# BUBLET/uav-airvision

Hardware: AMD Instinct MI355X
Metric: stereo frames/sec (LK+stereo+MSCKF-update) at 752x480 (higher is better)
Workload: dtype u8/int32 windows, f32 normal equations

## Files before the change

### include/airvision.h

```cpp
#ifndef AIRVISION_H
#define AIRVISION_H

#include <stddef.h>
#include <stdint.h>

#ifdef __cplusplus
extern "C" {
#endif

#define AV_OK            0
#define AV_E_INVALID    -1
#define AV_E_HIP        -2
#define AV_E_CAPACITY   -3
#define AV_E_NODEVICE   -4
#define AV_E_NUMERIC    -5

#define AV_MAX_LEVELS    5
#define AV_PYR_BORDER   16
#define AV_MAX_IMAGE_PIXELS (1 << 24)

const char* av_last_error(void);
const char* av_version(void);
int av_device_count(void);

typedef struct av_pyr_layout {
    int32_t levels;
    int32_t w[AV_MAX_LEVELS], h[AV_MAX_LEVELS];
    int32_t pitch[AV_MAX_LEVELS];
    int64_t offset[AV_MAX_LEVELS];
    int64_t bytes;
} av_pyr_layout;

int av_pyramid_layout(int w, int h, int levels, av_pyr_layout* out);

int av_pyramid_build(const uint8_t* img_dev, int64_t img_stride, int n_img, int w, int h, int levels,
                     uint8_t* pyr_dev, int64_t pyr_stride, void* stream);

int av_lk_track(const uint8_t* pyrI_dev, const uint8_t* pyrJ_dev, int64_t pyr_stride, int n_set,
                int w, int h, int levels,
                const float* prev_dev, float* next_dev, uint8_t* status_dev, const int32_t* count_dev, int cap,
                int win, int max_iter, double eps, double min_eig_threshold, void* stream);

int av_fast_detect(const uint8_t* img_dev, int64_t img_stride, const uint8_t* mask_dev, int64_t mask_stride,
                   int n_img, int w, int h, int threshold, uint32_t* kp_dev, int32_t* count_dev, int cap,
                   void* stream);
int av_fast_detect_wide(const uint8_t* img_dev, int64_t img_stride, const uint8_t* mask_dev, int64_t mask_stride,
                        int n_img, int w, int h, int threshold, uint32_t* kp_dev, int32_t* count_dev, int cap,
                        void* stream);

int av_undistort_points(const double* pts_dev, int n, const double* intr, const double* dist, const double* R,
                        double* out_dev, void* stream);
int av_distort_points(const double* pts_dev, int n, const double* intr, const double* dist,
                      double* out_dev, void* stream);

#define AV_DISTORTION_RADTAN 0
#define AV_DISTORTION_EQUIDISTANT 1
int av_undistort_points_model(const double* pts_dev, int n, const double* intr, const double* dist, const double* R, int model,
                              double* out_dev, void* stream);
int av_distort_points_model(const double* pts_dev, int n, const double* intr, const double* dist, int model,
                            double* out_dev, void* stream);

typedef struct av_frontend_config {
    int32_t width, height;
    int32_t grid_row, grid_col;
    int32_t grid_min_feature_num;
    int32_t grid_max_feature_num;
    int32_t fast_threshold;
    int32_t lk_win;
    int32_t lk_levels;
    int32_t lk_max_iter;
    int32_t max_corners;
    int32_t flags;
    double  lk_eps;
    double  lk_min_eig;
    double  stereo_threshold;
    double  cam0_intrinsics[4], cam0_distortion[4];
    double  cam1_intrinsics[4], cam1_distortion[4];
    double  R_cam0_imu[9], R_cam1_imu[9];
    double  R0to1[9];
    double  E[9];
    double  norm_unit;
    int32_t cam0_distortion_model;
    int32_t cam1_distortion_model;
    double  ransac_threshold;
    double  ransac_success_probability;
    uint32_t ransac_seed;
    int32_t reserved0;
    double  clahe_clip_limit;
    int32_t clahe_tiles_x, clahe_tiles_y;
    int32_t pixel_format;
    int32_t gray16_shift;
    int32_t image_downscale;
    int32_t reserved1;
} av_frontend_config;

typedef struct av_frontend av_frontend;

int  av_frontend_create(const av_frontend_config* cfg, int n_streams, int device, av_frontend** out);
void av_frontend_destroy(av_frontend* fe);

int av_frontend_push_imu(av_frontend* fe, int stream, double timestamp, const double gyro[3]);

int av_frontend_push_imu_batch(av_frontend* fe, const int32_t* stream_idx, const double* timestamps,
                               const double* gyro, int n);

#define AV_FE_INPUTS_PERSIST 1
#define AV_FE_RANSAC 2
#define AV_FE_CLAHE 4



int av_frontend_set_masks(av_frontend* fe, const uint8_t* mask0_host, const uint8_t* mask1_host);
int av_frontend_read_mask(av_frontend* fe, int cam, uint8_t* out_host);

#define AV_FE_PHOTOMETRIC 8
#define AV_PHOTOMETRIC_RESPONSE_MAX 65280
int av_frontend_set_photometric(av_frontend* fe, const uint16_t* response0_host, const uint16_t* gain0_host,
                                const uint16_t* response1_host, const uint16_t* gain1_host);
int av_frontend_read_photometric(av_frontend* fe, int cam, uint16_t* response_out_host, uint16_t* gain_out_host);

int av_frontend_step(av_frontend* fe, const uint8_t* img0_dev, const uint8_t* img1_dev, int64_t img_stride,
                     const double* timestamps, void* stream);
int av_frontend_prestage(av_frontend* fe, const uint8_t* img0_dev, const uint8_t* img1_dev, int64_t img_stride, void* stream);

int av_frontend_step_host(av_frontend* fe, const uint8_t* img0_host, const uint8_t* img1_host, int64_t img_stride,
                          const double* timestamps, void* stream);

int av_frontend_frames_reserve(av_frontend* fe, int n_slots);
int av_frontend_frames_upload(av_frontend* fe, const int32_t* slots, int n, const uint8_t* img0_host, const uint8_t* img1_host,
                              int64_t img_stride, void* stream);
int av_frontend_step_frames(av_frontend* fe, const int32_t* slot_of_stream, const double* timestamps, void* stream);

int av_png_decode_gray8(const char* const* paths, int n, int width, int height, uint8_t* out, int64_t out_stride, int threads, int32_t* status);
int av_png_decode(const char* const* paths, int n, int width, int height, int pixel_format, void* out, int64_t out_stride_bytes, int threads,
                  int32_t* status);
int av_png_probe(const char* path, int32_t* width, int32_t* height, int32_t* pixel_format);

int av_frontend_max_features(const av_frontend* fe);

int av_frontend_read_features(av_frontend* fe, int64_t* ids_out, double* uv_out, int32_t* n_out, int cap, void* stream);
int av_frontend_read_features_begin(av_frontend* fe, int slot, void* stream);
int av_frontend_read_features_end(av_frontend* fe, int slot, int64_t* ids_out, double* uv_out, int32_t* n_out, int cap);
int av_frontend_features_dev(av_frontend* fe, const int64_t** ids_dev, const double** uv_dev, const int32_t** n_dev, int* cap);

int av_frontend_read_grid(av_frontend* fe, int stream_idx, int64_t* ids, int32_t* lifetime, int32_t* cell,
                          float* pts, int cap, int32_t* n_out, int64_t* next_feature_id, void* stream);

int av_frontend_read_counters(av_frontend* fe, int stream_idx, int32_t out[8], void* stream);
int av_frontend_read_match_counts(av_frontend* fe, int stream_idx, int32_t out[2], void* stream);

int av_frontend_read_ransac_counts(av_frontend* fe, int stream_idx, int32_t out[4], void* stream);

int av_frontend_read_image(av_frontend* fe, int stream_idx, int cam, uint8_t* out_host, void* stream);

#define AV_CLAHE_MAX_TILES 16
int av_clahe(const uint8_t* img_dev, int64_t img_stride, int n_img, int w, int h, double clip_limit, int tiles_x, int tiles_y,
             uint8_t* out_dev, int64_t out_stride, uint8_t* lut_dev, void* stream);

#define AV_PIX_GRAY8  0
#define AV_PIX_GRAY16 1
#define AV_PIX_RGB8   2
#define AV_PIX_BGR8   3
#define AV_PIX_RGBA8  4
#define AV_PIX_BGRA8  5
#define AV_PIX_BAYER_RGGB8  16
#define AV_PIX_BAYER_BGGR8  17
#define AV_PIX_BAYER_GRBG8  18
#define AV_PIX_BAYER_GBRG8  19
#define AV_PIX_BAYER_RGGB16 20
#define AV_PIX_BAYER_BGGR16 21
#define AV_PIX_BAYER_GRBG16 22
#define AV_PIX_BAYER_GBRG16 23
#define AV_PIX_GRAY10P      32
#define AV_PIX_GRAY12P      33
#define AV_PIX_GRAY10_CSI2  34
#define AV_PIX_GRAY12_CSI2  35
#define AV_PIX_BAYER_RGGB10P     40
#define AV_PIX_BAYER_BGGR10P     41
#define AV_PIX_BAYER_GRBG10P     42
#define AV_PIX_BAYER_GBRG10P     43
#define AV_PIX_BAYER_RGGB12P     44
#define AV_PIX_BAYER_BGGR12P     45
#define AV_PIX_BAYER_GRBG12P     46
#define AV_PIX_BAYER_GBRG12P     47
#define AV_PIX_BAYER_RGGB10_CSI2 48
#define AV_PIX_BAYER_BGGR10_CSI2 49
#define AV_PIX_BAYER_GRBG10_CSI2 50
#define AV_PIX_BAYER_GBRG10_CSI2 51
#define AV_PIX_BAYER_RGGB12_CSI2 52
#define AV_PIX_BAYER_BGGR12_CSI2 53
#define AV_PIX_BAYER_GRBG12_CSI2 54
#define AV_PIX_BAYER_GBRG12_CSI2 55
int av_to_gray8(const void* img_dev, int64_t img_stride_bytes, int n_img, int w, int h, int pixel_format, int shift,
                uint8_t* out_dev, int64_t out_stride, void* stream);
int64_t av_pixfmt_frame_bytes(int pixel_format, int w, int h);

#define AV_GRAY16_SHIFT  0
#define AV_GRAY16_WINDOW 1
#define AV_GRAY16_AUTO   2
#define AV_GRAY16_MAX_CLIP_PPM 500000
#define AV_GRAY16_WORK_WORDS 4100
int av_to_gray8_range(const void* img_dev, int64_t img_stride_bytes, int n_img, int w, int h, int mode, int lo, int hi,
                      int ppm_lo, int ppm_hi, int min_span, int pool, const int32_t* index_dev,
                      uint8_t* out_dev, int64_t out_stride, int32_t* range_dev, uint32_t* work_dev, void* stream);
int av_frontend_set_gray16_scale(av_frontend* fe, int scale, int lo, int hi, int clip_lo_ppm, int clip_hi_ppm, int min_span);
int av_frontend_read_range(av_frontend* fe, int32_t* range_out_host, void* stream);

int av_downscale(const uint8_t* img_dev, int64_t img_stride, int n_img, int W, int H, int factor,
                 uint8_t* out_dev, int64_t out_stride, void* stream);
int av_downscale_vector_path(const uint8_t* img_dev, int64_t img_stride, int n_img, int W, int factor, const uint8_t* out_dev, int64_t out_stride);

int av_photometric(const uint8_t* in_dev, uint8_t* out_dev, int n, int w, int h, int64_t in_stride, int64_t out_stride,
                   const uint16_t* response_dev, const uint16_t* gain_dev, void* stream);
int av_photometric_vector_path(const uint8_t* in_dev, uint8_t* out_dev, int n, int w, int h, int64_t in_stride, int64_t out_stride,
                               const uint16_t* response_dev, const uint16_t* gain_dev);

#define AV_RANSAC_MAX_PAIRS       1920
#define AV_RANSAC_MAX_HYPOTHESES  64
#define AV_RANSAC_PATH_FEW    1
#define AV_RANSAC_PATH_STILL  2
#define AV_RANSAC_PATH_MODEL  4
#define AV_RANSAC_PATH_NONE   8
uint32_t av_ransac_hash(uint32_t seed, uint32_t frame, uint32_t camera, uint32_t k, uint32_t draw);
int av_ransac_num_hypotheses(double success_probability);
int av_two_point_ransac(const float* pts1_dev, const float* pts2_dev, const int32_t* off_dev, int n_problems, int max_pairs,
                        const double* R_dev, const int32_t* camera_dev, const int32_t* frame_dev,
                        const double* intr, const double* dist, int model, double inlier_error, double success_probability,
                        uint32_t seed, uint8_t* markers_dev, int32_t* info_dev, void* stream);

typedef struct av_msckf av_msckf;

int  av_msckf_create(int max_cam_states, int rows_cap, const double* chi2_table_100, int device, av_msckf** out);
void av_msckf_destroy(av_msckf* ctx);
int  av_msckf_ld(const av_msckf* ctx);
int  av_msckf_dim(const av_msckf* ctx);
int  av_msckf_set_cov(av_msckf* ctx, const double* P_host, int n, void* stream);
int  av_msckf_get_cov(av_msckf* ctx, double* P_host, int n, void* stream);
int  av_msckf_propagate(av_msckf* ctx, double dt, const double gyro[3], const double acc[3], const double q_old[4],
                        const double q_new[4], const double q_null[4], const double v_null[3], const double p_null[3],
                        const double v_new[3], const double p_new[3], const double gravity[3], const double noise[4],
                        void* stream);
int  av_msckf_augment(av_msckf* ctx, const double R_imu_cam0[9], const double skew_Rt_t[9], void* stream);
int  av_msckf_remove_cam(av_msckf* ctx, int cam_index, void* stream);
int  av_msckf_triangulate(av_msckf* ctx, int n_feat, const int32_t* obs_off_dev, const int32_t* obs_cam_dev, const double* obs_z_dev,
                          const double* cam_q_dev, const double* cam_p_dev, const double* T_cam0_cam1_rowmajor44,
                          const double* opt5, int max_views, double* pos_dev, int32_t* valid_dev, void* stream);
int  av_msckf_feature_blocks(av_msckf* ctx, int n_feat, int n_cam, int max_obs, const int32_t* obs_off_dev, const int32_t* obs_cam_dev,
                             const double* obs_z_dev, const double* pos_dev, const int32_t* dof_dev, const int32_t* row_off_dev, int total_rows,
                             const double* cam_q_dev, const double* cam_p_dev, const double* cam_qn_dev, const double* cam_pn_dev,
                             const double* T_cam0_cam1_rowmajor44, const double gravity[3], double obs_noise,
                             double* gamma_dev, int32_t* pass_dev, void* stream);
int  av_msckf_update(av_msckf* ctx, const int32_t* blk_row_dev, const int32_t* blk_len_dev, int n_blk, int total_rows,
                     double obs_noise, double* dx_host, void* stream);

int  av_quat_to_rotation(const double q[4], double R_rowmajor9[9]);
int  av_rotation_to_quat(const double R_rowmajor9[9], double q[4]);
int  av_quat_multiply(const double q1[4], const double q2[4], double out[4]);
int  av_quat_small_angle(const double dtheta[3], double q[4]);
int  av_quat_from_two_vectors(const double v0[3], const double v1[3], double q[4]);

typedef struct av_msckf_batch av_msckf_batch;
int  av_msckf_batch_create(int n_streams, int max_cam_states, int rows_cap, const double* chi2_table_100, const double gravity[3],
                           const double* T_cam0_cam1_rowmajor44, const double* R_imu_cam0_t_cam0_imu12, const double cov_init5[5],
                           const double noise4[4], double obs_noise, double position_std_threshold, const double velocity0[3],
                           const double* opt6, int device, av_msckf_batch** out);
void av_msckf_batch_destroy(av_msckf_batch* b);
int  av_msckf_batch_push_imu(av_msckf_batch* b, const int32_t* stream_idx, const double* timestamps, const double* gyro, const double* acc, int n);
int  av_msckf_batch_step(av_msckf_batch* b, const int64_t* ids, const double* uv, const int32_t* n_feat, int cap,
                         const double* timestamps, double* out, void* stream);
int  av_msckf_batch_submit(av_msckf_batch* b, const int64_t* ids, const double* uv, const int32_t* n_feat, int cap,
                           const double* timestamps, double* out, void* stream);
int  av_msckf_batch_wait(av_msckf_batch* b, int max_pending);
int  av_msckf_batch_device_resident(const av_msckf_batch* b);
int  av_msckf_batch_submit_dev(av_msckf_batch* b, const int64_t* ids_dev, const double* uv_dev, const int32_t* n_feat_dev, int cap,
                               const double* timestamps, double* out, void* msg_stream, void* stream);
int  av_msckf_batch_get_cov(av_msckf_batch* b, int stream_idx, double* P_host, int n, void* stream);
int  av_msckf_batch_sizes(av_msckf_batch* b, int stream_idx, int32_t out3[3]);
int  av_msckf_batch_get_state(av_msckf_batch* b, int stream_idx, double imu32[32], int64_t* cam_ids, double* cam_qp7, int cam_cap, int32_t* n_cam);
int  av_msckf_batch_stream_status(av_msckf_batch* b, int stream_idx, int32_t* status, char* msg, int msg_cap);
int  av_msckf_batch_counters(av_msckf_batch* b, int64_t out8[8]);
int  av_msckf_batch_debug_capture(av_msckf_batch* b, int enable);
int  av_msckf_batch_debug_read(av_msckf_batch* b, int stream_idx, int phase, double* gamma, int gamma_cap, int32_t* n_gamma,
                               double* dx, double* P_after, int n_cap, int32_t* n_state, int32_t* rows);
int  av_msckf_batch_work(av_msckf_batch* b, int enable, double out8[8]);
int  av_msckf_batch_work_executed(av_msckf_batch* b, double out2[2]);

int av_frontend_enable_timing(av_frontend* fe, int max_spans);
int av_frontend_read_timing(av_frontend* fe, double ms_out[4], int32_t spans_out[4]);

#ifdef __cplusplus
}
#endif
#endif
```

### uav_airvision_amd/_native.py

```python
import ctypes as C
import numbers
import os

import torch

_HERE = os.path.dirname(os.path.abspath(__file__))
LIB_PATH = os.path.join(_HERE, 'libairvision_hip.so')

AV_MAX_LEVELS = 5
AV_PYR_BORDER = 16
AV_MAX_IMAGE_PIXELS = 1 << 24
AV_OK, AV_E_INVALID, AV_E_HIP, AV_E_CAPACITY, AV_E_NODEVICE, AV_E_NUMERIC = 0, -1, -2, -3, -4, -5
AV_FE_INPUTS_PERSIST = 1
AV_FE_RANSAC = 2
AV_FE_CLAHE = 4
AV_FE_PHOTOMETRIC = 8
AV_PHOTOMETRIC_RESPONSE_MAX = 65280
AV_CLAHE_MAX_TILES = 16
AV_GRAY16_SHIFT, AV_GRAY16_WINDOW, AV_GRAY16_AUTO = 0, 1, 2
GRAY16_SCALES = {'shift': AV_GRAY16_SHIFT, 'window': AV_GRAY16_WINDOW, 'auto': AV_GRAY16_AUTO}
AV_GRAY16_MAX_CLIP_PPM = 500000
AV_GRAY16_WORK_WORDS = 4100
AV_PIX_GRAY8, AV_PIX_GRAY16, AV_PIX_RGB8, AV_PIX_BGR8, AV_PIX_RGBA8, AV_PIX_BGRA8 = 0, 1, 2, 3, 4, 5
AV_PIX_BAYER_RGGB8, AV_PIX_BAYER_BGGR8, AV_PIX_BAYER_GRBG8, AV_PIX_BAYER_GBRG8 = 16, 17, 18, 19
AV_PIX_BAYER_RGGB16, AV_PIX_BAYER_BGGR16, AV_PIX_BAYER_GRBG16, AV_PIX_BAYER_GBRG16 = 20, 21, 22, 23
AV_PIX_GRAY10P, AV_PIX_GRAY12P, AV_PIX_GRAY10_CSI2, AV_PIX_GRAY12_CSI2 = 32, 33, 34, 35
AV_PIX_BAYER_RGGB10P, AV_PIX_BAYER_RGGB12P, AV_PIX_BAYER_RGGB10_CSI2, AV_PIX_BAYER_RGGB12_CSI2 = 40, 44, 48, 52
AV_RANSAC_MAX_PAIRS = 1920
AV_RANSAC_MAX_HYPOTHESES = 64
AV_RANSAC_PATH_FEW, AV_RANSAC_PATH_STILL, AV_RANSAC_PATH_MODEL, AV_RANSAC_PATH_NONE = 1, 2, 4, 8


PIXEL_FORMATS = {'gray8': 0, 'gray16': 1, 'rgb8': 2, 'bgr8': 3, 'rgba8': 4, 'bgra8': 5,
                 'bayer_rggb8': 16, 'bayer_bggr8': 17, 'bayer_grbg8': 18, 'bayer_gbrg8': 19,
                 'bayer_rggb16': 20, 'bayer_bggr16': 21, 'bayer_grbg16': 22, 'bayer_gbrg16': 23}
BAYER_PATTERNS = ('rggb', 'bggr', 'grbg', 'gbrg')
PACKINGS = ('10p', '12p', '10_csi2', '12_csi2')
PACKED_FORMATS = dict([('gray' + k, 32 + i) for i, k in enumerate(PACKINGS)] +
                      [('bayer_%s%s' % (p, k), 40 + 4 * i + j) for i, k in enumerate(PACKINGS) for j, p in enumerate(BAYER_PATTERNS)])
PIXEL_FORMAT_NAMES = {v: k for k, v in list(PIXEL_FORMATS.items()) + list(PACKED_FORMATS.items())}
PIXEL_BYTES = {0: 1, 1: 2, 2: 3, 3: 3, 4: 4, 5: 4, 16: 1, 17: 1, 18: 1, 19: 1, 20: 2, 21: 2, 22: 2, 23: 2}


def is_packed(fmt):
    return AV_PIX_GRAY10P <= fmt <= AV_PIX_GRAY12_CSI2 or AV_PIX_BAYER_RGGB10P <= fmt <= AV_PIX_BAYER_RGGB12_CSI2 + 3


def packed_depth(fmt):
    if not is_packed(fmt):
        return 0
    return 12 if ((fmt - 32) if fmt < 40 else (fmt - 40) >> 2) & 1 else 10


def packing(fmt):
    if not is_packed(fmt):
        raise ValueError('%r is no packed format' % (fmt,))
    return PACKINGS[(fmt - 32) if fmt < 40 else (fmt - 40) >> 2]


def packed_group(fmt):
    return (4, 5) if packed_depth(fmt) == 10 else (2, 3)


def frame_bytes(fmt, w, h):
    return int(lib().av_pixfmt_frame_bytes(int(fmt), int(w), int(h)))


def packed_row_bytes(fmt, width):
    gpx, gb = packed_group(fmt)
    if not is_packed(fmt) or width <= 0 or width % gpx:
        raise ValueError('%s: a row is whole groups of %d samples, width %d is not' % (PIXEL_FORMAT_NAMES.get(fmt, fmt), gpx, width))
    return width // gpx * gb


def is_bayer(fmt):
    return AV_PIX_BAYER_RGGB8 <= fmt <= AV_PIX_BAYER_GBRG16 or AV_PIX_BAYER_RGGB10P <= fmt <= AV_PIX_BAYER_RGGB12_CSI2 + 3


def is_16bit(fmt):
    return fmt == AV_PIX_GRAY16 or AV_PIX_BAYER_RGGB16 <= fmt <= AV_PIX_BAYER_GBRG16


def pixel_format_code(name):
    if isinstance(name, str) and name in PIXEL_FORMATS:
        return PIXEL_FORMATS[name]
    if isinstance(name, str) and name in PACKED_FORMATS:
        return PACKED_FORMATS[name]
    if isinstance(name, int) and not isinstance(name, bool) and name in PIXEL_FORMAT_NAMES:
        return name
    raise ValueError('unknown image format %r (one of %s)' % (name, ', '.join(PIXEL_FORMAT_NAMES[c] for c in sorted(PIXEL_FORMAT_NAMES))))


def gray16_shift_value(shift):
    if isinstance(shift, bool) or int(shift) != shift or not 0 <= int(shift) <= 8:
        raise ValueError('gray16_shift %r outside 0 .. 8' % (shift,))
    return int(shift)


def _int_in(v, lo, hi):
    return not isinstance(v, bool) and isinstance(v, numbers.Real) and int(v) == v and lo <= int(v) <= hi


def gray16_range_settings(scale='shift', window=None, clip=(100, 100), min_span=256):
    if scale not in GRAY16_SCALES:
        raise ValueError("gray16_scale %r is none of 'shift', 'window', 'auto'" % (scale,))
    mode, lo, hi, ppm, span = GRAY16_SCALES[scale], 0, 65535, (100, 100), 256
    if mode == AV_GRAY16_WINDOW:
        try:
            lo, hi = window
        except (TypeError, ValueError):
            raise ValueError("gray16_scale 'window' needs gray16_window = (lo, hi), got %r" % (window,))
        if not (_int_in(lo, 0, 65535) and _int_in(hi, 0, 65535) and lo < hi):
            raise ValueError('gray16_window %r does not satisfy 0 <= lo < hi <= 65535' % (window,))
    if mode == AV_GRAY16_AUTO:
        try:
            ppm = tuple(clip)
        except TypeError:
            ppm = ()
        if len(ppm) != 2 or not all(_int_in(v, 0, AV_GRAY16_MAX_CLIP_PPM) for v in ppm) or sum(ppm) > AV_GRAY16_MAX_CLIP_PPM:
            raise ValueError('gray16_auto_clip %r: two integers >= 0 in parts per million whose sum is at most %d' % (clip, AV_GRAY16_MAX_CLIP_PPM))
        if not _int_in(min_span, 16, 65535):
            raise ValueError('gray16_auto_min_span %r outside 16 .. 65535' % (min_span,))
        span = min_span
    return mode, int(lo), int(hi), int(ppm[0]), int(ppm[1]), int(span)


def downscale_value(factor):
    if isinstance(factor, bool) or not isinstance(factor, numbers.Real) or int(factor) != factor or int(factor) not in (1, 2, 4):
        raise ValueError('image_downscale %r is none of 1, 2, 4' % (factor,))
    return int(factor)


DISTORTION_MODELS = {'radtan': 0, 'equidistant': 1}


def distortion_model_code(name):
    return 1 if name == 'equidistant' else 0


class AirvisionError(RuntimeError):
    def __init__(self, code, text):
        RuntimeError.__init__(self, 'libairvision_hip error %d: %s' % (code, text))
        self.code = code


class PyrLayout(C.Structure):
    _fields_ = [('levels', C.c_int32),
                ('w', C.c_int32 * AV_MAX_LEVELS), ('h', C.c_int32 * AV_MAX_LEVELS),
                ('pitch', C.c_int32 * AV_MAX_LEVELS),
                ('offset', C.c_int64 * AV_MAX_LEVELS),
                ('bytes', C.c_int64)]


class FrontendConfig(C.Structure):
    _fields_ = [('width', C.c_int32), ('height', C.c_int32),
                ('grid_row', C.c_int32), ('grid_col', C.c_int32),
                ('grid_min_feature_num', C.c_int32), ('grid_max_feature_num', C.c_int32),
                ('fast_threshold', C.c_int32), ('lk_win', C.c_int32), ('lk_levels', C.c_int32),
                ('lk_max_iter', C.c_int32), ('max_corners', C.c_int32), ('flags', C.c_int32),
                ('lk_eps', C.c_double), ('lk_min_eig', C.c_double), ('stereo_threshold', C.c_double),
                ('cam0_intrinsics', C.c_double * 4), ('cam0_distortion', C.c_double * 4),
                ('cam1_intrinsics', C.c_double * 4), ('cam1_distortion', C.c_double * 4),
                ('R_cam0_imu', C.c_double * 9), ('R_cam1_imu', C.c_double * 9),
                ('R0to1', C.c_double * 9), ('E', C.c_double * 9), ('norm_unit', C.c_double),
                ('cam0_distortion_model', C.c_int32), ('cam1_distortion_model', C.c_int32),
                ('ransac_threshold', C.c_double), ('ransac_success_probability', C.c_double),
                ('ransac_seed', C.c_uint32), ('reserved0', C.c_int32),
                ('clahe_clip_limit', C.c_double), ('clahe_tiles_x', C.c_int32), ('clahe_tiles_y', C.c_int32),
                ('pixel_format', C.c_int32), ('gray16_shift', C.c_int32),
                ('image_downscale', C.c_int32), ('reserved1', C.c_int32)]


_P = C.c_void_p
SIGNATURES = {
    'av_last_error': (C.c_char_p, []),
    'av_version': (C.c_char_p, []),
    'av_device_count': (C.c_int, []),
    'av_pyramid_layout': (C.c_int, [C.c_int, C.c_int, C.c_int, C.POINTER(PyrLayout)]),
    'av_pyramid_build': (C.c_int, [_P, C.c_int64, C.c_int, C.c_int, C.c_int, C.c_int, _P, C.c_int64, _P]),
    'av_lk_track': (C.c_int, [_P, _P, C.c_int64, C.c_int, C.c_int, C.c_int, C.c_int, _P, _P, _P, _P, C.c_int,
                              C.c_int, C.c_int, C.c_double, C.c_double, _P]),
    'av_fast_detect': (C.c_int, [_P, C.c_int64, _P, C.c_int64, C.c_int, C.c_int, C.c_int, C.c_int, _P, _P, C.c_int, _P]),
    'av_fast_detect_wide': (C.c_int, [_P, C.c_int64, _P, C.c_int64, C.c_int, C.c_int, C.c_int, C.c_int, _P, _P, C.c_int, _P]),
    'av_undistort_points': (C.c_int, [_P, C.c_int, C.POINTER(C.c_double), C.POINTER(C.c_double), C.POINTER(C.c_double), _P, _P]),
    'av_distort_points': (C.c_int, [_P, C.c_int, C.POINTER(C.c_double), C.POINTER(C.c_double), _P, _P]),
    'av_undistort_points_model': (C.c_int, [_P, C.c_int, C.POINTER(C.c_double), C.POINTER(C.c_double), C.POINTER(C.c_double), C.c_int, _P, _P]),
    'av_distort_points_model': (C.c_int, [_P, C.c_int, C.POINTER(C.c_double), C.POINTER(C.c_double), C.c_int, _P, _P]),
    'av_frontend_create': (C.c_int, [C.POINTER(FrontendConfig), C.c_int, C.c_int, C.POINTER(_P)]),
    'av_frontend_destroy': (None, [_P]),
    'av_frontend_push_imu': (C.c_int, [_P, C.c_int, C.c_double, C.POINTER(C.c_double)]),
    'av_frontend_push_imu_batch': (C.c_int, [_P, _P, _P, _P, C.c_int]),
    'av_frontend_step': (C.c_int, [_P, _P, _P, C.c_int64, C.POINTER(C.c_double), _P]),
    'av_frontend_prestage': (C.c_int, [_P, _P, _P, C.c_int64, _P]),
    'av_frontend_step_host': (C.c_int, [_P, _P, _P, C.c_int64, C.POINTER(C.c_double), _P]),
    'av_frontend_frames_reserve': (C.c_int, [_P, C.c_int]),
    'av_frontend_frames_upload': (C.c_int, [_P, _P, C.c_int, _P, _P, C.c_int64, _P]),
    'av_frontend_step_frames': (C.c_int, [_P, _P, C.POINTER(C.c_double), _P]),
    'av_frontend_max_features': (C.c_int, [_P]),
    'av_frontend_read_features': (C.c_int, [_P, _P, _P, _P, C.c_int, _P]),
    'av_frontend_read_features_begin': (C.c_int, [_P, C.c_int, _P]),
    'av_frontend_features_dev': (C.c_int, [_P, _P, _P, _P, _P]),
    'av_frontend_read_features_end': (C.c_int, [_P, C.c_int, _P, _P, _P, C.c_int]),
    'av_frontend_read_grid': (C.c_int, [_P, C.c_int, _P, _P, _P, _P, C.c_int, C.POINTER(C.c_int32), C.POINTER(C.c_int64), _P]),
    'av_frontend_read_counters': (C.c_int, [_P, C.c_int, C.POINTER(C.c_int32 * 8), _P]),
    'av_frontend_read_match_counts': (C.c_int, [_P, C.c_int, C.POINTER(C.c_int32 * 2), _P]),
    'av_msckf_create': (C.c_int, [C.c_int, C.c_int, C.POINTER(C.c_double), C.c_int, C.POINTER(_P)]),
    'av_msckf_destroy': (None, [_P]),
    'av_msckf_ld': (C.c_int, [_P]),
    'av_msckf_dim': (C.c_int, [_P]),
    'av_msckf_set_cov': (C.c_int, [_P, _P, C.c_int, _P]),
    'av_msckf_get_cov': (C.c_int, [_P, _P, C.c_int, _P]),
    'av_msckf_propagate': (C.c_int, [_P, C.c_double] + [C.POINTER(C.c_double)] * 11 + [_P]),
    'av_msckf_augment': (C.c_int, [_P, C.POINTER(C.c_double), C.POINTER(C.c_double), _P]),
    'av_msckf_remove_cam': (C.c_int, [_P, C.c_int, _P]),
    'av_msckf_triangulate': (C.c_int, [_P, C.c_int, _P, _P, _P, _P, _P, C.POINTER(C.c_double), C.POINTER(C.c_double), C.c_int, _P, _P, _P]),
    'av_msckf_feature_blocks': (C.c_int, [_P, C.c_int, C.c_int, C.c_int, _P, _P, _P, _P, _P, _P, C.c_int, _P, _P, _P, _P,
                                          C.POINTER(C.c_double), C.POINTER(C.c_double), C.c_double, _P, _P, _P]),
    'av_msckf_update': (C.c_int, [_P, _P, _P, C.c_int, C.c_int, C.c_double, _P, _P]),
    'av_msckf_batch_create': (C.c_int, [C.c_int, C.c_int, C.c_int] + [C.POINTER(C.c_double)] * 6 + [C.c_double, C.c_double, C.POINTER(C.c_double), C.POINTER(C.c_double), C.c_int, C.POINTER(_P)]),
    'av_msckf_batch_destroy': (None, [_P]),
    'av_msckf_batch_push_imu': (C.c_int, [_P, _P, _P, _P, _P, C.c_int]),
    'av_msckf_batch_step': (C.c_int, [_P, _P, _P, _P, C.c_int, _P, _P, _P]),
    'av_msckf_batch_submit': (C.c_int, [_P, _P, _P, _P, C.c_int, _P, _P, _P]),
    'av_msckf_batch_device_resident': (C.c_int, [_P]),
    'av_msckf_batch_submit_dev': (C.c_int, [_P, _P, _P, _P, C.c_int, _P, _P, _P, _P]),
    'av_msckf_batch_wait': (C.c_int, [_P, C.c_int]),
    'av_msckf_batch_get_cov': (C.c_int, [_P, C.c_int, _P, C.c_int, _P]),
    'av_msckf_batch_sizes': (C.c_int, [_P, C.c_int, C.POINTER(C.c_int32 * 3)]),
    'av_msckf_batch_counters': (C.c_int, [_P, C.POINTER(C.c_int64 * 8)]),
    'av_png_decode_gray8': (C.c_int, [_P, C.c_int, C.c_int, C.c_int, _P, C.c_int64, C.c_int, _P]),
    'av_png_decode': (C.c_int, [_P, C.c_int, C.c_int, C.c_int, C.c_int, _P, C.c_int64, C.c_int, _P]),
    'av_png_probe': (C.c_int, [C.c_char_p, C.POINTER(C.c_int32), C.POINTER(C.c_int32), C.POINTER(C.c_int32)]),
    'av_to_gray8': (C.c_int, [_P, C.c_int64, C.c_int, C.c_int, C.c_int, C.c_int, C.c_int, _P, C.c_int64, _P]),
    'av_pixfmt_frame_bytes': (C.c_int64, [C.c_int, C.c_int, C.c_int]),
    'av_to_gray8_range': (C.c_int, [_P, C.c_int64] + [C.c_int] * 10 + [_P, _P, C.c_int64, _P, _P, _P]),
    'av_frontend_set_gray16_scale': (C.c_int, [_P] + [C.c_int] * 6),
    'av_frontend_read_range': (C.c_int, [_P, _P, _P]),
    'av_downscale': (C.c_int, [_P, C.c_int64, C.c_int, C.c_int, C.c_int, C.c_int, _P, C.c_int64, _P]),
    'av_downscale_vector_path': (C.c_int, [_P, C.c_int64, C.c_int, C.c_int, C.c_int, _P, C.c_int64]),
    'av_quat_to_rotation': (C.c_int, [_P, _P]),
    'av_rotation_to_quat': (C.c_int, [_P, _P]),
    'av_quat_multiply': (C.c_int, [_P, _P, _P]),
    'av_quat_small_angle': (C.c_int, [_P, _P]),
    'av_quat_from_two_vectors': (C.c_int, [_P, _P, _P]),
    'av_msckf_batch_debug_capture': (C.c_int, [_P, C.c_int]),
    'av_msckf_batch_debug_read': (C.c_int, [_P, C.c_int, C.c_int, _P, C.c_int, C.POINTER(C.c_int32), _P, _P, C.c_int, C.POINTER(C.c_int32), C.POINTER(C.c_int32)]),
    'av_msckf_batch_work': (C.c_int, [_P, C.c_int, C.POINTER(C.c_double * 8)]),
    'av_msckf_batch_work_executed': (C.c_int, [_P, C.POINTER(C.c_double * 2)]),
    'av_msckf_batch_get_state': (C.c_int, [_P, C.c_int, C.POINTER(C.c_double * 32), _P, _P, C.c_int, C.POINTER(C.c_int32)]),
    'av_msckf_batch_stream_status': (C.c_int, [_P, C.c_int, C.POINTER(C.c_int32), C.c_char_p, C.c_int]),
    'av_frontend_read_ransac_counts': (C.c_int, [_P, C.c_int, C.POINTER(C.c_int32 * 4), _P]),
    'av_ransac_hash': (C.c_uint32, [C.c_uint32] * 5),
    'av_ransac_num_hypotheses': (C.c_int, [C.c_double]),
    'av_two_point_ransac': (C.c_int, [_P, _P, _P, C.c_int, C.c_int, _P, _P, _P, C.POINTER(C.c_double), C.POINTER(C.c_double), C.c_int,
                                      C.c_double, C.c_double, C.c_uint32, _P, _P, _P]),
    'av_frontend_read_image': (C.c_int, [_P, C.c_int, C.c_int, _P, _P]),
    'av_clahe': (C.c_int, [_P, C.c_int64, C.c_int, C.c_int, C.c_int, C.c_double, C.c_int, C.c_int, _P, C.c_int64, _P, _P]),
    'av_frontend_set_masks': (C.c_int, [_P, _P, _P]),
    'av_frontend_read_mask': (C.c_int, [_P, C.c_int, _P]),
    'av_frontend_set_photometric': (C.c_int, [_P, _P, _P, _P, _P]),
    'av_frontend_read_photometric': (C.c_int, [_P, C.c_int, _P, _P]),
    'av_photometric': (C.c_int, [_P, _P, C.c_int, C.c_int, C.c_int, C.c_int64, C.c_int64, _P, _P, _P]),
    'av_photometric_vector_path': (C.c_int, [_P, _P, C.c_int, C.c_int, C.c_int, C.c_int64, C.c_int64, _P, _P]),
    'av_frontend_enable_timing': (C.c_int, [_P, C.c_int]),
    'av_frontend_read_timing': (C.c_int, [_P, C.POINTER(C.c_double * 4), C.POINTER(C.c_int32 * 4)]),
}

_lib = None


def lib():
    global _lib
    if _lib is None:
        if not os.path.exists(LIB_PATH):
            raise RuntimeError('libairvision_hip.so is not built (%s); run `python -m uav_airvision_amd.build` -- '
                               'there is no CPU fallback' % LIB_PATH)
        l = C.CDLL(LIB_PATH)
        for name, (res, args) in SIGNATURES.items():
            fn = getattr(l, name)
            fn.restype = res
            fn.argtypes = args
        _lib = l
    return _lib


def check(rc):
    if rc != 0:
        raise AirvisionError(rc, lib().av_last_error().decode('utf-8', 'replace'))


def current_stream():
    return C.c_void_p(torch.cuda.current_stream().cuda_stream)


def dptr(t):
    return C.c_void_p(t.data_ptr())


def darr(a):
    return (C.c_double * len(a))(*[float(v) for v in a])
```

### uav_airvision_amd/csrc/pyramid.hip

```cpp
#include <limits.h>
#include <stdlib.h>

#include "av_common.h"

namespace {

struct PyrArgs {
    const uint8_t* img0;
    const uint8_t* img1;
    int64_t img_stride;
    int imgs_per_stream;
    uint8_t* pyr_base;
    int64_t stream_stride, slot_stride;
    int slot0, slot1;
    PyrGeom g;
    int n_img, tiles_x, tiles_y;
    const int* index;
};

__device__ __forceinline__ void pyr_entry(const PyrArgs& a, int img, int& s, int& cam)
{
    s = img / a.imgs_per_stream; cam = img - s * a.imgs_per_stream;
    if (a.index) s = a.index[s];
}

__device__ __forceinline__ uint8_t* pyr_of(const PyrArgs& a, int img)
{
    int s, cam;
    pyr_entry(a, img, s, cam);
    return a.pyr_base + s * a.stream_stride + (cam == 0 ? a.slot0 : a.slot1) * a.slot_stride;
}

__global__ __launch_bounds__(256) void pad_level0_kernel(PyrArgs a)
{
    const int w = a.g.w[0], h = a.g.h[0], pitch = a.g.pitch[0];
    const int chunks_per_row = pitch >> 4;
    const int ph = h + 2 * AV_PYR_BORDER;
    int q = blockIdx.x * blockDim.x + threadIdx.x;
    if (q >= chunks_per_row * ph) return;
    int yp = q / chunks_per_row, xc = q - yp * chunks_per_row;
    int img = blockIdx.y;
    int s, cam;
    pyr_entry(a, img, s, cam);
    const uint8_t* src = (cam == 0 ? a.img0 : a.img1) + s * a.img_stride;
    uint8_t* dst = pyr_of(a, img) + a.g.off[0];
    int y = av_reflect101(yp - AV_PYR_BORDER, h);
    const uint8_t* row = src + (size_t)y * w;
    const int x0 = xc * 16 - AV_PYR_BORDER;
    uint4 out;
    if (x0 >= 0 && x0 + 16 <= w && ((w | (int)(a.img_stride & 15) | (int)(reinterpret_cast<uintptr_t>(src) & 15)) & 15) == 0) {
        out = *reinterpret_cast<const uint4*>(row + x0);
    } else {
        uint32_t o[4] = {0, 0, 0, 0};
#pragma unroll
        for (int i = 0; i < 16; ++i) {
            int x = av_reflect101(x0 + i, w);
            x = min(max(x, 0), w - 1);
            o[i >> 2] |= (uint32_t)row[x] << (8 * (i & 3));
        }
        out = make_uint4(o[0], o[1], o[2], o[3]);
    }
    *reinterpret_cast<uint4*>(dst + (size_t)yp * pitch + xc * 16) = out;
}

constexpr int FT_W = 128, FT_LP = FT_W + 8;
constexpr int FT_H_TALL = 96, FT_H_BASE = 32;
template <bool WRITE_L0, int FT_H>
__global__ __launch_bounds__(256) void pyr_l0l1_kernel(PyrArgs a)
{
    __shared__ __attribute__((aligned(16))) uint8_t src[(FT_H + 4) * FT_LP];
    __shared__ __attribute__((aligned(16))) uint16_t hs[(FT_H + 4) * (FT_W / 2)];
    static_assert((FT_H / 2) * (FT_W / 2) <= (FT_H + 4) * FT_LP, "level-1 tile fits the source tile");
    uint8_t* const l1t = src;
    const int w = a.g.w[0], h = a.g.h[0], pitch0 = a.g.pitch[0];
    const int w1 = a.g.w[1], h1 = a.g.h[1], pitch1 = a.g.pitch[1];
    const int tid = threadIdx.x;
    const int L = blockIdx.x, wg = L >> 3, per = a.tiles_x * a.tiles_y;
    const int img = (L & 7) + 8 * (wg / per);
    if (img >= a.n_img) return;
    const int tile = wg % per;
    const int by = tile / a.tiles_x, bx = tile - by * a.tiles_x;
    const int x0 = bx * FT_W, y0 = by * FT_H;
    int s, cam;
    pyr_entry(a, img, s, cam);
    const uint8_t* in = (cam == 0 ? a.img0 : a.img1) + s * a.img_stride;
    uint8_t* base = pyr_of(a, img);
    uint8_t* d0 = base + a.g.off[0];
    uint8_t* d1 = base + a.g.off[1];
    uint32_t* srcw = reinterpret_cast<uint32_t*>(src);

    const bool al16 = ((a.img_stride & 15) == 0) && ((reinterpret_cast<uintptr_t>(in) & 15) == 0);
    {
        constexpr int NIT = ((FT_H + 4) * 10 + 255) / 256;
        uint4 q4[NIT]; uint32_t hv[NIT]; int kind[NIT], rr[NIT], jj[NIT];
#pragma unroll
        for (int u = 0; u < NIT; ++u) {
            const int i = tid + 256 * u;
            const bool valid = i < (FT_H + 4) * 10;
            const int r = valid ? i / 10 : 0, j = valid ? i - r * 10 : 0;
            rr[u] = r; jj[u] = j;
            kind[u] = valid ? 3 : 0; hv[u] = 0; q4[u] = make_uint4(0, 0, 0, 0);
        }
        if (al16) {
#pragma unroll
            for (int u = 0; u < NIT; ++u) {
                const int r = rr[u], j = jj[u];
                const uint8_t* row = in + (size_t)av_reflect101(y0 - 2 + r, h) * w;
                const int gx = x0 + 16 * j, gh = j == 8 ? x0 - 4 : x0 + FT_W;
                const bool ok16 = kind[u] != 0 && j < 8 && gx + 16 <= w;
                const bool okh = kind[u] != 0 && j >= 8 && gh >= 0 && gh + 4 <= w;
                q4[u] = *reinterpret_cast<const uint4*>(ok16 ? row + gx : in);
                hv[u] = *reinterpret_cast<const uint32_t*>(okh ? row + gh : in);
                kind[u] = ok16 ? 1 : (okh ? 2 : kind[u]);
            }
        }
#pragma unroll
        for (int u = 0; u < NIT; ++u) {
            const int r = rr[u], j = jj[u];
            if (kind[u] == 1) {
                uint32_t* dst = srcw + r * (FT_LP / 4) + 1 + 4 * j;
                dst[0] = q4[u].x; dst[1] = q4[u].y; dst[2] = q4[u].z; dst[3] = q4[u].w;
            } else if (kind[u] == 2) {
                srcw[r * (FT_LP / 4) + (j == 8 ? 0 : FT_LP / 4 - 1)] = hv[u];
            } else if (kind[u] == 3) {
                const uint8_t* row = in + (size_t)av_reflect101(y0 - 2 + r, h) * w;
                if (j < 8) {
                    const int gx = x0 + 16 * j;
                    uint32_t v[4];
#pragma unroll
                    for (int d = 0; d < 4; ++d) {
                        if (gx + 4 * d + 4 <= w) v[d] = *reinterpret_cast<const uint32_t*>(row + gx + 4 * d);
                        else {
                            v[d] = 0;
#pragma unroll
                            for (int b = 0; b < 4; ++b) { int x = av_reflect101(gx + 4 * d + b, w); x = min(max(x, 0), w - 1); v[d] |= (uint32_t)row[x] << (8 * b); }
                        }
                    }
                    uint32_t* dst = srcw + r * (FT_LP / 4) + 1 + 4 * j;
                    dst[0] = v[0]; dst[1] = v[1]; dst[2] = v[2]; dst[3] = v[3];
                } else {
                    const int gx = j == 8 ? x0 - 4 : x0 + FT_W;
                    uint32_t v = 0;
#pragma unroll
                    for (int b = 0; b < 4; ++b) { int x = av_reflect101(gx + b, w); x = min(max(x, 0), w - 1); v |= (uint32_t)row[x] << (8 * b); }
                    srcw[r * (FT_LP / 4) + (j == 8 ? 0 : FT_LP / 4 - 1)] = v;
                }
            }
        }
    }
    __syncthreads();

    if (WRITE_L0) {
        const bool top = y0 == 0, bot = y0 + FT_H >= h, left = x0 == 0, right = x0 + FT_W >= w;
        const int tw = min(FT_W, w - x0);
        const int nrow = FT_H + (top ? AV_PYR_BORDER : 0) + (bot ? AV_PYR_BORDER : 0);
        const int nch_in = (tw + 15) >> 4;
        const int nch = nch_in + (left ? 1 : 0) + (right ? (pitch0 - AV_PYR_BORDER - w + 15) / 16 : 0);
        for (int i = tid; i < nrow * nch; i += 256) {
            const int ri = i / nch, ci = i - ri * nch;
            int yp;
            if (ri < FT_H) yp = y0 + ri;
            else if (top && ri < FT_H + AV_PYR_BORDER) yp = -(ri - FT_H + 1);
            else yp = h + (ri - FT_H - (top ? AV_PYR_BORDER : 0));
            if (yp >= h + AV_PYR_BORDER || (ri < FT_H && yp >= h)) continue;
            int xd;
            bool interior;
            if (ci < nch_in) { xd = x0 + 16 * ci; interior = true; }
            else if (left && ci == nch_in) { xd = -AV_PYR_BORDER; interior = false; }
            else { xd = w + 16 * (ci - nch_in - (left ? 1 : 0)); interior = false; }
            const int sy = av_reflect101(yp, h) - (y0 - 2);
            uint32_t o[4];
            if (interior && xd + 16 <= w) {
                const uint32_t* p = srcw + sy * (FT_LP / 4) + ((xd - x0 + 4) >> 2);
                o[0] = p[0]; o[1] = p[1]; o[2] = p[2]; o[3] = p[3];
            } else {
                o[0] = o[1] = o[2] = o[3] = 0;
#pragma unroll
                for (int b = 0; b < 16; ++b) {
                    int x = av_reflect101(xd + b, w); x = min(max(x, 0), w - 1);
                    o[b >> 2] |= (uint32_t)src[sy * FT_LP + (x - x0 + 4)] << (8 * (b & 3));
                }
            }
            *reinterpret_cast<uint4*>(d0 + (size_t)(yp + AV_PYR_BORDER) * pitch0 + (xd + AV_PYR_BORDER)) = make_uint4(o[0], o[1], o[2], o[3]);
        }
    }

    for (int i = tid; i < (FT_H + 4) * (FT_W / 8); i += 256) {
        const int r = i / (FT_W / 8), xq = i - r * (FT_W / 8);
        const uint2 lo = *reinterpret_cast<const uint2*>(src + r * FT_LP + 8 * xq);
        const uint2 hi = *reinterpret_cast<const uint2*>(src + r * FT_LP + 8 * xq + 8);
        const uint32_t dx_ = lo.x, dy_ = lo.y, dz_ = hi.x, dw_ = hi.y;
        const uint32_t t0 = __builtin_amdgcn_alignbyte(dy_, dx_, 2), t1 = dy_, t2 = __builtin_amdgcn_alignbyte(dz_, dy_, 2), t3 = dz_;
        const uint32_t W4 = 0x04060401u;
        const uint32_t h0 = __builtin_amdgcn_udot4(t0, W4, (dy_ >> 16) & 0xFF, false);
        const uint32_t h1_ = __builtin_amdgcn_udot4(t1, W4, dz_ & 0xFF, false);
        const uint32_t h2 = __builtin_amdgcn_udot4(t2, W4, (dz_ >> 16) & 0xFF, false);
        const uint32_t h3 = __builtin_amdgcn_udot4(t3, W4, dw_ & 0xFF, false);
        *reinterpret_cast<uint2*>(hs + r * (FT_W / 2) + 4 * xq) = make_uint2(h0 | (h1_ << 16), h2 | (h3 << 16));
    }
    __syncthreads();
    for (int t_ = tid; t_ < (FT_H / 2) * (FT_W / 8); t_ += 256) {
        const int yo = t_ >> 4, xq = t_ & 15;
        uint32_t out = 0;
        const uint16_t* c = hs + (2 * yo) * (FT_W / 2) + 4 * xq;
#pragma unroll
        for (int k = 0; k < 4; ++k) {
            const int v = (int)c[k] + (int)c[4 * (FT_W / 2) + k] + 4 * ((int)c[(FT_W / 2) + k] + (int)c[3 * (FT_W / 2) + k]) + 6 * (int)c[2 * (FT_W / 2) + k];
            out |= (uint32_t)((v + 128) >> 8) << (8 * k);
        }
        *reinterpret_cast<uint32_t*>(l1t + yo * (FT_W / 2) + 4 * xq) = out;
        const int x1 = x0 / 2 + 4 * xq, y1 = y0 / 2 + yo;
        if (x1 < w1 && y1 < h1) *reinterpret_cast<uint32_t*>(d1 + (size_t)(y1 + AV_PYR_BORDER) * pitch1 + (x1 + AV_PYR_BORDER)) = out;
    }
    const int X1 = x0 / 2, Y1 = y0 / 2;
    const bool band = X1 <= AV_PYR_BORDER || X1 + FT_W / 2 >= w1 - AV_PYR_BORDER - 1 || Y1 <= AV_PYR_BORDER || Y1 + FT_H / 2 >= h1 - AV_PYR_BORDER - 1;
    if (band) {
        __syncthreads();
        for (int i = tid; i < (FT_H / 2) * (FT_W / 2); i += 256) {
            const int yo = i / (FT_W / 2), xo = i - yo * (FT_W / 2);
            const int x1 = X1 + xo, y1 = Y1 + yo;
            if (x1 >= w1 || y1 >= h1) continue;
            const uint8_t v = l1t[i];
            const int xm = (x1 >= 1 && x1 <= AV_PYR_BORDER) ? -x1 : ((x1 >= w1 - 1 - AV_PYR_BORDER && x1 <= w1 - 2) ? 2 * (w1 - 1) - x1 : INT_MIN);
            const int ym = (y1 >= 1 && y1 <= AV_PYR_BORDER) ? -y1 : ((y1 >= h1 - 1 - AV_PYR_BORDER && y1 <= h1 - 2) ? 2 * (h1 - 1) - y1 : INT_MIN);
            if (xm != INT_MIN) d1[(size_t)(y1 + AV_PYR_BORDER) * pitch1 + (xm + AV_PYR_BORDER)] = v;
            if (ym != INT_MIN) d1[(size_t)(ym + AV_PYR_BORDER) * pitch1 + (x1 + AV_PYR_BORDER)] = v;
            if (xm != INT_MIN && ym != INT_MIN) d1[(size_t)(ym + AV_PYR_BORDER) * pitch1 + (xm + AV_PYR_BORDER)] = v;
        }
    }
}

__global__ __launch_bounds__(256) void pyr_down_kernel(PyrArgs a, int level)
{
    const int w = a.g.w[level], h = a.g.h[level], pitch = a.g.pitch[level];
    const int spitch = a.g.pitch[level - 1];
    const int quads_per_row = pitch >> 2;
    const int ph = h + 2 * AV_PYR_BORDER;
    int q = blockIdx.x * blockDim.x + threadIdx.x;
    if (q >= quads_per_row * ph) return;
    int yp = q / quads_per_row, xq = q - yp * quads_per_row;
    uint8_t* base = pyr_of(a, blockIdx.y);
    const uint8_t* src = base + a.g.off[level - 1];
    uint8_t* dst = base + a.g.off[level];
    int y = av_reflect101(yp - AV_PYR_BORDER, h);
    const uint8_t* r0 = src + (size_t)(2 * y - 2 + AV_PYR_BORDER) * spitch + AV_PYR_BORDER;
    uint32_t out = 0;
    const int x0 = xq * 4 - AV_PYR_BORDER;
    if (x0 >= 0 && x0 + 4 <= w) {
        int hs[4][5];
#pragma unroll
        for (int k = 0; k < 5; ++k) {
            const uint4 d = *reinterpret_cast<const uint4*>(r0 + (size_t)k * spitch + 2 * x0 - 4);
            const uint32_t t0 = __builtin_amdgcn_alignbyte(d.y, d.x, 2), t1 = d.y, t2 = __builtin_amdgcn_alignbyte(d.z, d.y, 2), t3 = d.z;
            const uint32_t W4 = 0x04060401u;
            hs[0][k] = (int)__builtin_amdgcn_udot4(t0, W4, (d.y >> 16) & 0xFF, false);
            hs[1][k] = (int)__builtin_amdgcn_udot4(t1, W4, d.z & 0xFF, false);
            hs[2][k] = (int)__builtin_amdgcn_udot4(t2, W4, (d.z >> 16) & 0xFF, false);
            hs[3][k] = (int)__builtin_amdgcn_udot4(t3, W4, d.w & 0xFF, false);
        }
#pragma unroll
        for (int i = 0; i < 4; ++i) {
            const int v = hs[i][0] + hs[i][4] + 4 * (hs[i][1] + hs[i][3]) + 6 * hs[i][2];
            out |= (uint32_t)((v + 128) >> 8) << (8 * i);
        }
    } else {
#pragma unroll
        for (int i = 0; i < 4; ++i) {
            int xp = xq * 4 + i;
            int x = av_reflect101(xp - AV_PYR_BORDER, w);
            x = min(max(x, 0), w - 1);
            const uint8_t* p = r0 + 2 * x;
            int hsum[5];
#pragma unroll
            for (int k = 0; k < 5; ++k) {
                const uint8_t* r = p + (size_t)k * spitch;
                hsum[k] = (int)r[-2] + (int)r[2] + 4 * ((int)r[-1] + (int)r[1]) + 6 * (int)r[0];
            }
            int v = hsum[0] + hsum[4] + 4 * (hsum[1] + hsum[3]) + 6 * hsum[2];
            out |= (uint32_t)((v + 128) >> 8) << (8 * i);
        }
    }
    *reinterpret_cast<uint32_t*>(dst + (size_t)yp * pitch + xq * 4) = out;
}

template <int L23_T>
__global__ __launch_bounds__(L23_T) void pyr_l2l3_kernel(PyrArgs a)
{
    extern __shared__ uint8_t lds23[];
    const int w1 = a.g.w[1], p1 = a.g.pitch[1];
    const int w2 = a.g.w[2], h2 = a.g.h[2], p2 = a.g.pitch[2];
    const int w3 = a.g.w[3], h3 = a.g.h[3], p3 = a.g.pitch[3];
    const int lp2 = (w2 + 3) & ~3, lp3 = (w3 + 3) & ~3;
    uint8_t* l2 = lds23;
    uint8_t* l3 = lds23 + (((size_t)h2 * lp2 + 15) & ~(size_t)15);
    const int tid = threadIdx.x;
    uint8_t* base = pyr_of(a, blockIdx.x);
    const uint8_t* s1 = base + a.g.off[1] + (size_t)AV_PYR_BORDER * p1 + AV_PYR_BORDER;
    uint8_t* d2 = base + a.g.off[2];
    uint8_t* d3 = base + a.g.off[3];
    (void)w1;
    const int q2 = lp2 >> 2;
    for (int i = tid; i < q2 * h2; i += L23_T) {
        const int y = i / q2, x0 = (i - y * q2) * 4;
        const uint8_t* r0 = s1 + (ptrdiff_t)(2 * y - 2) * p1;
        int hs[4][5];
#pragma unroll
        for (int k = 0; k < 5; ++k) {
            const uint4 d = *reinterpret_cast<const uint4*>(r0 + (size_t)k * p1 + 2 * x0 - 4);
            const uint32_t t0 = __builtin_amdgcn_alignbyte(d.y, d.x, 2), t1 = d.y, t2 = __builtin_amdgcn_alignbyte(d.z, d.y, 2), t3 = d.z;
            const uint32_t W4 = 0x04060401u;
            hs[0][k] = (int)__builtin_amdgcn_udot4(t0, W4, (d.y >> 16) & 0xFF, false);
            hs[1][k] = (int)__builtin_amdgcn_udot4(t1, W4, d.z & 0xFF, false);
            hs[2][k] = (int)__builtin_amdgcn_udot4(t2, W4, (d.z >> 16) & 0xFF, false);
            hs[3][k] = (int)__builtin_amdgcn_udot4(t3, W4, d.w & 0xFF, false);
        }
        uint32_t out = 0;
#pragma unroll
        for (int c = 0; c < 4; ++c) {
            const int v = hs[c][0] + hs[c][4] + 4 * (hs[c][1] + hs[c][3]) + 6 * hs[c][2];
            out |= (uint32_t)((v + 128) >> 8) << (8 * c);
        }
        *reinterpret_cast<uint32_t*>(l2 + y * lp2 + x0) = out;
    }
    __syncthreads();
    const int ph2 = h2 + 2 * AV_PYR_BORDER, pq2 = p2 >> 2;
    for (int i = tid; i < pq2 * ph2; i += L23_T) {
        const int yp = i / pq2, xq = i - yp * pq2;
        const int y = av_reflect101(yp - AV_PYR_BORDER, h2);
        uint32_t out = 0;
        const int xs = xq * 4 - AV_PYR_BORDER;
        if (xs >= 0 && xs + 4 <= w2) out = *reinterpret_cast<const uint32_t*>(l2 + y * lp2 + xs);
        else {
#pragma unroll
            for (int c = 0; c < 4; ++c) { int x = av_reflect101(xs + c, w2); x = min(max(x, 0), w2 - 1); out |= (uint32_t)l2[y * lp2 + x] << (8 * c); }
        }
        *reinterpret_cast<uint32_t*>(d2 + (size_t)yp * p2 + xq * 4) = out;
    }
    const int q3 = lp3 >> 2;
    for (int i = tid; i < q3 * h3; i += L23_T) {
        const int y = i / q3, x0 = (i - y * q3) * 4;
        uint32_t out = 0;
#pragma unroll
        for (int c = 0; c < 4; ++c) {
            const int x = x0 + c;
            int v = 0;
            if (x < w3) {
                int hsum[5];
#pragma unroll
                for (int k = 0; k < 5; ++k) {
                    const uint8_t* r = l2 + av_reflect101(2 * y - 2 + k, h2) * lp2;
                    const int xm2 = av_reflect101(2 * x - 2, w2), xm1 = av_reflect101(2 * x - 1, w2), xp1 = av_reflect101(2 * x + 1, w2), xp2 = av_reflect101(2 * x + 2, w2);
                    hsum[k] = (int)r[xm2] + (int)r[xp2] + 4 * ((int)r[xm1] + (int)r[xp1]) + 6 * (int)r[2 * x];
                }
                v = (hsum[0] + hsum[4] + 4 * (hsum[1] + hsum[3]) + 6 * hsum[2] + 128) >> 8;
            }
            out |= (uint32_t)v << (8 * c);
        }
        *reinterpret_cast<uint32_t*>(l3 + y * lp3 + x0) = out;
    }
    __syncthreads();
    const int ph3 = h3 + 2 * AV_PYR_BORDER, pq3 = p3 >> 2;
    for (int i = tid; i < pq3 * ph3; i += L23_T) {
        const int yp = i / pq3, xq = i - yp * pq3;
        const int y = av_reflect101(yp - AV_PYR_BORDER, h3);
        uint32_t out = 0;
        const int xs = xq * 4 - AV_PYR_BORDER;
        if (xs >= 0 && xs + 4 <= w3) out = *reinterpret_cast<const uint32_t*>(l3 + y * lp3 + xs);
        else {
#pragma unroll
            for (int c = 0; c < 4; ++c) { int x = av_reflect101(xs + c, w3); x = min(max(x, 0), w3 - 1); out |= (uint32_t)l3[y * lp3 + x] << (8 * c); }
        }
        *reinterpret_cast<uint32_t*>(d3 + (size_t)yp * p3 + xq * 4) = out;
    }
}

}

PyrGeom av_make_geom(const av_pyr_layout& l)
{
    PyrGeom g;
    memset(&g, 0, sizeof(g));
    g.levels = l.levels;
    for (int i = 0; i < l.levels; ++i) {
        g.w[i] = l.w[i]; g.h[i] = l.h[i]; g.pitch[i] = l.pitch[i]; g.off[i] = (int)l.offset[i];
    }
    return g;
}

int av_launch_pyramid(const FrameSet& img, int n_groups,
                      const PyrGeom& g, uint8_t* pyr_base, int64_t stream_stride, int64_t slot_stride, int slot0, int slot1,
                      hipStream_t st, bool write_level0, bool* wrote_level0)
{
    if (wrote_level0) *wrote_level0 = true;
    if (n_groups <= 0) return AV_OK;
    PyrArgs a;
    a.img0 = img.base[0]; a.img1 = img.base[1]; a.img_stride = img.stride; a.imgs_per_stream = img.base[1] ? 2 : 1;
    a.pyr_base = pyr_base; a.stream_stride = stream_stride; a.slot_stride = slot_stride;
    a.slot0 = slot0; a.slot1 = slot1; a.g = g;
    a.n_img = 0; a.tiles_x = 0; a.tiles_y = 0; a.index = img.map;
    const int n_img = n_groups * a.imgs_per_stream;
    const int w = g.w[0], h = g.h[0];
    const int FT_H = ((h % FT_H_TALL) == 0 && h >= 2 * FT_H_TALL) ? FT_H_TALL : FT_H_BASE;
    const bool fused = g.levels >= 2 && (w & 15) == 0 && (h % FT_H) == 0 && h >= 64 && w >= 64 && (w % FT_W == 0 || w % FT_W >= 20) &&
                       (img.stride & 3) == 0 && (reinterpret_cast<uintptr_t>(img.base[0]) & 3) == 0 && (reinterpret_cast<uintptr_t>(img.base[1]) & 3) == 0;
    if (fused) {
        const int tx = (w + FT_W - 1) / FT_W, ty = h / FT_H;
        a.n_img = n_img; a.tiles_x = tx; a.tiles_y = ty;
        dim3 grid((unsigned)(tx * ty) * 8u * (unsigned)((n_img + 7) / 8));
        if (FT_H == FT_H_TALL) {
            if (write_level0) hipLaunchKernelGGL((pyr_l0l1_kernel<true, FT_H_TALL>), grid, dim3(256), 0, st, a);
            else { hipLaunchKernelGGL((pyr_l0l1_kernel<false, FT_H_TALL>), grid, dim3(256), 0, st, a); if (wrote_level0) *wrote_level0 = false; }
        } else {
            if (write_level0) hipLaunchKernelGGL((pyr_l0l1_kernel<true, FT_H_BASE>), grid, dim3(256), 0, st, a);
            else { hipLaunchKernelGGL((pyr_l0l1_kernel<false, FT_H_BASE>), grid, dim3(256), 0, st, a); if (wrote_level0) *wrote_level0 = false; }
        }
        AV_LAUNCH_CHECK();
    } else {
        int chunks = (g.pitch[0] >> 4) * (g.h[0] + 2 * AV_PYR_BORDER);
        dim3 grid((chunks + 255) / 256, n_img);
        hipLaunchKernelGGL(pad_level0_kernel, grid, dim3(256), 0, st, a);
        AV_LAUNCH_CHECK();
    }
    const size_t lds23 = g.levels == 4 ? ((((size_t)g.h[2] * ((g.w[2] + 3) & ~3) + 15) & ~(size_t)15) + (size_t)g.h[3] * ((g.w[3] + 3) & ~3) + 16) : 0;
    const bool fused23 = g.levels == 4 && lds23 <= 60 * 1024 && (g.pitch[1] & 3) == 0;
    int lbeg = fused ? 2 : 1;
    if (fused23) {
        if (!fused) {
            int quads = (g.pitch[1] >> 2) * (g.h[1] + 2 * AV_PYR_BORDER);
            dim3 grid((quads + 255) / 256, n_img);
            hipLaunchKernelGGL(pyr_down_kernel, grid, dim3(256), 0, st, a, 1);
            AV_LAUNCH_CHECK();
        }
        hipLaunchKernelGGL(pyr_l2l3_kernel<1024>, dim3(n_img), dim3(1024), lds23, st, a);
        AV_LAUNCH_CHECK();
        lbeg = g.levels;
    }
    for (int l = lbeg; l < g.levels; ++l) {
        int quads = (g.pitch[l] >> 2) * (g.h[l] + 2 * AV_PYR_BORDER);
        dim3 grid((quads + 255) / 256, n_img);
        hipLaunchKernelGGL(pyr_down_kernel, grid, dim3(256), 0, st, a, l);
        AV_LAUNCH_CHECK();
    }
    return AV_OK;
}

AV_EXPORT int av_pyramid_layout(int w, int h, int levels, av_pyr_layout* out)
{
    if (!out || levels < 1 || levels > AV_MAX_LEVELS || w <= 0 || h <= 0) {
        av_set_error("av_pyramid_layout: bad arguments (w=%d h=%d levels=%d)", w, h, levels);
        return AV_E_INVALID;
    }
    memset(out, 0, sizeof(*out));
    out->levels = levels;
    int64_t off = 0;
    int lw = w, lh = h;
    for (int l = 0; l < levels; ++l) {
        if (lw <= AV_PYR_BORDER || lh <= AV_PYR_BORDER) {
            av_set_error("av_pyramid_layout: level %d is %dx%d, too small for a %d-pixel reflect-101 frame", l, lw, lh, AV_PYR_BORDER);
            return AV_E_INVALID;
        }
        out->w[l] = lw; out->h[l] = lh;
        out->pitch[l] = ((lw + 2 * AV_PYR_BORDER) + 15) & ~15;
        out->offset[l] = off;
        off += (int64_t)out->pitch[l] * (lh + 2 * AV_PYR_BORDER);
        lw = (lw + 1) / 2; lh = (lh + 1) / 2;
    }
    out->bytes = (off + 255) & ~(int64_t)255;
    if (out->bytes > 0x7fffffff) { av_set_error("av_pyramid_layout: image too large"); return AV_E_INVALID; }
    return AV_OK;
}

AV_EXPORT int av_pyramid_build(const uint8_t* img_dev, int64_t img_stride, int n_img, int w, int h, int levels,
                               uint8_t* pyr_dev, int64_t pyr_stride, void* stream)
{
    av_pyr_layout lay;
    int rc = av_pyramid_layout(w, h, levels, &lay);
    if (rc) return rc;
    if (!img_dev || !pyr_dev || n_img < 0 || pyr_stride < lay.bytes || img_stride < (int64_t)w * h) {
        av_set_error("av_pyramid_build: bad arguments");
        return AV_E_INVALID;
    }
    return av_launch_pyramid(av_frames(img_dev, nullptr, img_stride), n_img, av_make_geom(lay), pyr_dev, pyr_stride, 0, 0, 0, (hipStream_t)stream);
}
```

### uav_airvision_amd/ops.py

```python
import ctypes as C

import numpy as np
import torch

from . import _native as N


def _dev(device):
    return torch.device('cuda', device)


def pyramid_layout(w, h, levels):
    lay = N.PyrLayout()
    N.check(N.lib().av_pyramid_layout(w, h, levels, C.byref(lay)))
    return lay


def build_pyramids(images, levels, device=0):
    t = torch.as_tensor(images)
    if t.dim() == 2:
        t = t[None]
    t = t.to(_dev(device), dtype=torch.uint8).contiguous()
    n, h, w = t.shape
    lay = pyramid_layout(w, h, levels)
    pyr = torch.empty((n, lay.bytes), dtype=torch.uint8, device=_dev(device))
    with torch.cuda.device(device):
        N.check(N.lib().av_pyramid_build(N.dptr(t), w * h, n, w, h, levels, N.dptr(pyr), lay.bytes, N.current_stream()))
    return pyr, lay


def pyramid_level(pyr_row, lay, level, with_border=False):
    a = pyr_row.cpu().numpy()
    B = N.AV_PYR_BORDER
    w, h, pitch, off = lay.w[level], lay.h[level], lay.pitch[level], lay.offset[level]
    full = a[off:off + pitch * (h + 2 * B)].reshape(h + 2 * B, pitch)
    return full[:, :w + 2 * B] if with_border else full[B:B + h, B:B + w]


def calc_optical_flow_pyr_lk(prev_img, next_img, prev_pts, next_pts, winSize=(15, 15), maxLevel=3,
                             criteria=(3, 30, 0.01), flags=4, minEigThreshold=1e-4, device=0):
    if not (flags & 4):
        raise ValueError('only OPTFLOW_USE_INITIAL_FLOW is implemented (the reference always sets it)')
    ctype, max_iter, eps = criteria
    max_iter = int(max_iter) if (ctype & 1) else 30
    eps = float(eps) if (ctype & 2) else 0.01
    prev = np.ascontiguousarray(np.asarray(prev_pts, dtype=np.float32).reshape(-1, 2))
    nxt = np.ascontiguousarray(np.asarray(next_pts, dtype=np.float32).reshape(-1, 2))
    n = prev.shape[0]
    if n == 0:
        return nxt.copy(), np.zeros((0, 1), np.uint8), None
    imgs = np.stack([np.asarray(prev_img, dtype=np.uint8), np.asarray(next_img, dtype=np.uint8)])
    lw, lh, eff = imgs.shape[2], imgs.shape[1], 0
    while eff < maxLevel and (lw + 1) // 2 > winSize[0] and (lh + 1) // 2 > winSize[1]:
        lw, lh, eff = (lw + 1) // 2, (lh + 1) // 2, eff + 1
    maxLevel = eff
    pyr, lay = build_pyramids(imgs, maxLevel + 1, device)
    dev = _dev(device)
    d_prev = torch.from_numpy(prev).to(dev)
    d_next = torch.from_numpy(nxt).to(dev)
    d_status = torch.zeros(n, dtype=torch.uint8, device=dev)
    d_count = torch.tensor([n], dtype=torch.int32, device=dev)
    h, w = imgs.shape[1:]
    with torch.cuda.device(device):
        N.check(N.lib().av_lk_track(N.dptr(pyr[0]), N.dptr(pyr[1]), lay.bytes, 1, w, h, maxLevel + 1,
                                    N.dptr(d_prev), N.dptr(d_next), N.dptr(d_status), N.dptr(d_count), n,
                                    int(winSize[0]), max_iter, eps, float(minEigThreshold), N.current_stream()))
        torch.cuda.synchronize()
    return d_next.cpu().numpy(), d_status.cpu().numpy().reshape(-1, 1), None


KP_RASTER_BITS, KP_RASTER_BITS_WIDE = 19, 24


def kp_raster_bits(w, h):
    if w * h > N.AV_MAX_IMAGE_PIXELS:
        raise ValueError('fast_detect: %d x %d exceeds AV_MAX_IMAGE_PIXELS = 2^24 pixels' % (w, h))
    return KP_RASTER_BITS if w * h <= (1 << KP_RASTER_BITS) else KP_RASTER_BITS_WIDE


def pack_keypoints(x, y, score, w, bits):
    raster = np.asarray(y, np.int64) * int(w) + np.asarray(x, np.int64)
    score = np.asarray(score, np.int64)
    if raster.size and (raster.min() < 0 or raster.max() >= (1 << bits) or score.min() < 0 or (score.max() << bits) >= (1 << 32)):
        raise ValueError('pack_keypoints: raster or score outside the %d-bit format' % bits)
    return ((score << bits) | (((1 << bits) - 1) - raster)).astype(np.uint32)


def unpack_keypoints(words, w, bits):
    words = np.asarray(words).view(np.uint32)
    m = np.uint32((1 << bits) - 1)
    raster = (m - (words & m)).astype(np.int64)
    score = (words >> np.uint32(bits)).astype(np.int32)
    order = np.argsort(raster, kind='stable')
    raster, score = raster[order], score[order]
    return (raster % w).astype(np.int32), (raster // w).astype(np.int32), score


def fast_detect(img, threshold, mask=None, cap=1 << 16, device=0):
    dev = _dev(device)
    t = torch.as_tensor(np.ascontiguousarray(img, dtype=np.uint8)).to(dev)
    h, w = t.shape
    bits = kp_raster_bits(w, h)
    entry = N.lib().av_fast_detect if bits == KP_RASTER_BITS else N.lib().av_fast_detect_wide
    m = None if mask is None else torch.as_tensor(np.ascontiguousarray(mask, dtype=np.uint8)).to(dev)
    kp = torch.empty(cap, dtype=torch.int32, device=dev)
    cnt = torch.zeros(1, dtype=torch.int32, device=dev)
    with torch.cuda.device(device):
        N.check(entry(N.dptr(t), w * h, None if m is None else N.dptr(m), w * h, 1, w, h, int(threshold),
                      N.dptr(kp), N.dptr(cnt), cap, N.current_stream()))
        torch.cuda.synchronize()
    n = int(cnt.item())
    if n > cap:
        raise N.AirvisionError(N.AV_E_CAPACITY, 'FAST found %d keypoints, capacity %d' % (n, cap))
    return unpack_keypoints(kp[:n].cpu().numpy(), w, bits)


def _points_op(fn_name, pts_in, extra, device):
    arr = np.asarray(pts_in)
    out_f32 = arr.dtype == np.float32
    pts = np.ascontiguousarray(arr.reshape(-1, 2), dtype=np.float64)
    n = pts.shape[0]
    if n == 0:
        return pts.astype(np.float32) if out_f32 else pts
    dev = _dev(device)
    d_in = torch.from_numpy(pts).to(dev)
    d_out = torch.empty_like(d_in)
    with torch.cuda.device(device):
        N.check(getattr(N.lib(), fn_name)(N.dptr(d_in), n, *extra, N.dptr(d_out), N.current_stream()))
        torch.cuda.synchronize()
    out = d_out.cpu().numpy()
    return out.astype(np.float32) if out_f32 else out


def undistort_points(pts_in, intrinsics, distortion_coeffs, rectification_matrix=None, device=0, distortion_model='radtan'):
    R = np.eye(3) if rectification_matrix is None else np.asarray(rectification_matrix, dtype=np.float64)
    extra = (N.darr(intrinsics), N.darr(distortion_coeffs), N.darr(R.reshape(-1)), N.distortion_model_code(distortion_model))
    return _points_op('av_undistort_points_model', pts_in, extra, device)


def distort_points(pts_in, intrinsics, distortion_coeffs, device=0, distortion_model='radtan'):
    extra = (N.darr(intrinsics), N.darr(distortion_coeffs), N.distortion_model_code(distortion_model))
    return _points_op('av_distort_points_model', pts_in, extra, device)


def ransac_num_hypotheses(success_probability=0.99):
    return int(N.lib().av_ransac_num_hypotheses(float(success_probability)))


def ransac_hash(seed, frame, camera, k, draw):
    return int(N.lib().av_ransac_hash(int(seed) & 0xFFFFFFFF, int(frame) & 0xFFFFFFFF, int(camera), int(k), int(draw)))


def two_point_ransac_batch(pts1, pts2, R_p_c, intrinsics, distortion_model, distortion_coeffs, inlier_error, success_probability=0.99,
                           seed=0, frames=None, cameras=None, device=0):
    B = len(pts1)
    assert len(pts2) == B
    p1 = [np.asarray(p, dtype=np.float32).reshape(-1, 2) for p in pts1]
    p2 = [np.asarray(p, dtype=np.float32).reshape(-1, 2) for p in pts2]
    sizes = [len(p) for p in p1]
    assert sizes == [len(p) for p in p2], 'pts1 and pts2 must pair up'
    if B == 0:
        return [], np.zeros((0, 2), np.int32)
    off = np.zeros(B + 1, np.int32)
    off[1:] = np.cumsum(sizes)
    total, max_pairs = int(off[-1]), max(sizes)
    if max_pairs > N.AV_RANSAC_MAX_PAIRS:
        raise ValueError('two_point_ransac: %d pairs in one problem, at most %d' % (max_pairs, N.AV_RANSAC_MAX_PAIRS))
    dev = _dev(device)
    cat = lambda ps: np.ascontiguousarray(np.concatenate(ps, axis=0)) if total else np.zeros((1, 2), np.float32)
    d1 = torch.from_numpy(cat(p1)).to(dev)
    d2 = torch.from_numpy(cat(p2)).to(dev)
    d_off = torch.from_numpy(off).to(dev)
    d_R = torch.from_numpy(np.ascontiguousarray(np.asarray(R_p_c, dtype=np.float64).reshape(B, 9))).to(dev)
    d_fr = torch.from_numpy(np.ascontiguousarray(np.zeros(B) if frames is None else frames, dtype=np.int64).astype(np.uint32).view(np.int32)).to(dev)
    d_cam = torch.from_numpy(np.ascontiguousarray(np.zeros(B) if cameras is None else cameras, dtype=np.int32)).to(dev)
    d_mark = torch.zeros(max(total, 1), dtype=torch.uint8, device=dev)
    d_info = torch.zeros((B, 2), dtype=torch.int32, device=dev)
    with torch.cuda.device(device):
        N.check(N.lib().av_two_point_ransac(N.dptr(d1), N.dptr(d2), N.dptr(d_off), B, max_pairs, N.dptr(d_R), N.dptr(d_cam), N.dptr(d_fr),
                                            N.darr(intrinsics), N.darr(distortion_coeffs), N.distortion_model_code(distortion_model),
                                            float(inlier_error), float(success_probability), int(seed) & 0xFFFFFFFF,
                                            N.dptr(d_mark), N.dptr(d_info), N.current_stream()))
        torch.cuda.synchronize()
    mark = d_mark.cpu().numpy()
    return [mark[off[b]:off[b + 1]].copy() for b in range(B)], d_info.cpu().numpy()


def two_point_ransac(pts1, pts2, R_p_c, intrinsics, distortion_model, distortion_coeffs, inlier_error, success_probability=0.99,
                     seed=0, frame=0, camera=0, device=0):
    marks, _info = two_point_ransac_batch([pts1], [pts2], [R_p_c], intrinsics, distortion_model, distortion_coeffs, inlier_error,
                                          success_probability, seed, [frame], [camera], device)
    return marks[0]


def clahe(img, clip_limit=2.0, tiles=(8, 8), out=None, return_lut=False, device=0):
    t = torch.as_tensor(img)
    if t.dtype != torch.uint8 or t.dim() not in (2, 3):
        raise ValueError('clahe: uint8 [n, h, w] or [h, w] images, got %s %s' % (t.dtype, tuple(t.shape)))
    t = t.to(_dev(device)).contiguous()
    shape = tuple(t.shape)
    h, w = shape[-2:]
    n = shape[0] if t.dim() == 3 else 1
    if out is None:
        out = torch.empty_like(t)
    elif not (out.is_cuda and out.dtype == torch.uint8 and tuple(out.shape) == shape and out.is_contiguous()):
        raise ValueError('clahe: out must be a contiguous uint8 cuda tensor of shape %s' % (shape,))
    tx, ty = [int(v) for v in tiles]
    lut = torch.empty((n, max(tx * ty, 1), 256), dtype=torch.uint8, device=_dev(device)) if return_lut else None
    with torch.cuda.device(device):
        N.check(N.lib().av_clahe(N.dptr(t), w * h, n, w, h, float(clip_limit), tx, ty, N.dptr(out), w * h,
                                 None if lut is None else N.dptr(lut), N.current_stream()))
    return (out, lut) if return_lut else out


def to_gray8(img, pixel_format, shift=8, out=None, device=0):
    fmt = N.pixel_format_code(pixel_format)
    shift = N.gray16_shift_value(shift)
    t = torch.as_tensor(img)
    if N.is_packed(fmt):
        return _packed_to_gray8(t, fmt, shift, out, device)
    bpp = N.PIXEL_BYTES[fmt]
    colour = bpp >= 3
    dtypes = (torch.uint16, torch.int16) if N.is_16bit(fmt) else (torch.uint8,)
    core = 3 if colour else 2
    if t.dtype not in dtypes or t.dim() not in (core, core + 1) or (colour and t.shape[-1] != bpp):
        raise ValueError('to_gray8: %s images are %s [n, h, w%s] or [h, w%s], got %s %s' % (
            N.PIXEL_FORMAT_NAMES[fmt], ' / '.join(str(d) for d in dtypes), ', %d' % bpp if colour else '', ', %d' % bpp if colour else '', t.dtype, tuple(t.shape)))
    if N.is_bayer(fmt) and (t.shape[-1] < 2 or t.shape[-2] < 2):
        raise ValueError('to_gray8: a Bayer mosaic is at least 2 x 2 samples, got %s' % (tuple(t.shape),))
    t = t.to(_dev(device))
    batched = t.dim() == core + 1
    tb = t if batched else t.unsqueeze(0)
    if not tb[0].is_contiguous():
        tb = tb.contiguous()
    n, h, w = tb.shape[0], tb.shape[1], tb.shape[2]
    if n > 1 and tb.stride(0) < h * w * (bpp if colour else 1):
        tb = tb.contiguous()
    oshape = (n, h, w) if batched else (h, w)
    if out is None:
        out = torch.empty(oshape, dtype=torch.uint8, device=_dev(device))
    elif not (isinstance(out, torch.Tensor) and out.is_cuda and out.dtype == torch.uint8 and tuple(out.shape) == oshape):
        raise ValueError('to_gray8: out must be a uint8 cuda tensor of shape %s' % (oshape,))
    ob = out if batched else out.unsqueeze(0)
    if not ob[0].is_contiguous() or (n > 1 and ob.stride(0) < h * w):
        raise ValueError('to_gray8: every image of out must be contiguous')
    in_stride = (tb.stride(0) if n > 1 else h * w * (bpp if colour else 1)) * tb.element_size()
    out_stride = ob.stride(0) if n > 1 else h * w
    with torch.cuda.device(device):
        N.check(N.lib().av_to_gray8(N.dptr(tb), in_stride, n, w, h, fmt, shift, N.dptr(ob), out_stride, N.current_stream()))
    return out


def _packed_to_gray8(t, fmt, shift, out, device):
    name, d = N.PIXEL_FORMAT_NAMES[fmt], N.packed_depth(fmt)
    gpx, gb = N.packed_group(fmt)
    if t.dtype != torch.uint8 or t.dim() not in (2, 3) or t.shape[-1] == 0 or t.shape[-1] % gb:
        raise ValueError('to_gray8: %s images are torch.uint8 [n, h, w * %d / 8] or [h, w * %d / 8] with rows of whole %d-byte groups, got %s %s' % (
            name, d, d, gb, t.dtype, tuple(t.shape)))
    wb = int(t.shape[-1])
    w = wb // gb * gpx
    if N.is_bayer(fmt) and (w < 2 or t.shape[-2] < 2):
        raise ValueError('to_gray8: a Bayer mosaic is at least 2 x 2 samples, got %s' % (tuple(t.shape),))
    t = t.to(_dev(device))
    batched = t.dim() == 3
    tb = t if batched else t.unsqueeze(0)
    n, h = tb.shape[0], tb.shape[1]
    if not tb[0].is_contiguous() or (n > 1 and tb.stride(0) < h * wb):
        tb = tb.contiguous()
    oshape = (n, h, w) if batched else (h, w)
    if out is None:
        out = torch.empty(oshape, dtype=torch.uint8, device=_dev(device))
    elif not (isinstance(out, torch.Tensor) and out.is_cuda and out.dtype == torch.uint8 and tuple(out.shape) == oshape):
        raise ValueError('to_gray8: out must be a uint8 cuda tensor of shape %s' % (oshape,))
    ob = out if batched else out.unsqueeze(0)
    if not ob[0].is_contiguous() or (n > 1 and ob.stride(0) < h * w):
        raise ValueError('to_gray8: every image of out must be contiguous')
    in_stride = tb.stride(0) if n > 1 else h * wb
    out_stride = ob.stride(0) if n > 1 else h * w
    with torch.cuda.device(device):
        N.check(N.lib().av_to_gray8(N.dptr(tb), in_stride, n, w, h, fmt, shift, N.dptr(ob), out_stride, N.current_stream()))
    return out


def downscale(img, factor, out=None, device=0):
    if isinstance(factor, bool) or factor not in (2, 4):
        raise ValueError('downscale: factor %r is neither 2 nor 4' % (factor,))
    f = int(factor)
    t = torch.as_tensor(img)
    if t.dtype != torch.uint8 or t.dim() not in (2, 3):
        raise ValueError('downscale: images are torch.uint8 [n, H, W] or [H, W], got %s %s' % (t.dtype, tuple(t.shape)))
    H, W = int(t.shape[-2]), int(t.shape[-1])
    if H == 0 or W == 0 or H % f or W % f:
        raise ValueError('downscale: %d x %d is not divisible by the factor %d' % (W, H, f))
    t = t.to(_dev(device))
    batched = t.dim() == 3
    tb = t if batched else t.unsqueeze(0)
    n = tb.shape[0]
    if (n and not tb[0].is_contiguous()) or (n > 1 and tb.stride(0) < H * W):
        tb = tb.contiguous()
    h, w = H // f, W // f
    oshape = (n, h, w) if batched else (h, w)
    if out is None:
        out = torch.empty(oshape, dtype=torch.uint8, device=_dev(device))
    elif not (isinstance(out, torch.Tensor) and out.is_cuda and out.dtype == torch.uint8 and tuple(out.shape) == oshape):
        raise ValueError('downscale: out must be a uint8 cuda tensor of shape %s' % (oshape,))
    ob = out if batched else out.unsqueeze(0)
    if (n and not ob[0].is_contiguous()) or (n > 1 and ob.stride(0) < h * w):
        raise ValueError('downscale: every image of out must be contiguous')
    in_stride = tb.stride(0) if n > 1 else H * W
    out_stride = ob.stride(0) if n > 1 else h * w
    with torch.cuda.device(device):
        N.check(N.lib().av_downscale(N.dptr(tb), in_stride, n, W, H, f, N.dptr(ob), out_stride, N.current_stream()))
    return out


def photometric(images, response=None, gain=None, out=None, device=0):
    t = torch.as_tensor(images)
    if t.dtype != torch.uint8 or t.dim() not in (2, 3):
        raise ValueError('photometric: images are torch.uint8 [n, h, w] or [h, w], got %s %s' % (t.dtype, tuple(t.shape)))
    if response is None and gain is None:
        raise ValueError('photometric: neither a response table nor a gain map')
    t = t.to(_dev(device))
    batched = t.dim() == 3
    tb = t if batched else t.unsqueeze(0)
    n, h, w = tb.shape
    if (n and not tb[0].is_contiguous()) or (n > 1 and tb.stride(0) < h * w):
        tb = tb.contiguous()

    def table(a, what, shape):
        if isinstance(a, torch.Tensor):
            ok = a.dtype in tuple(d for d in (getattr(torch, 'uint16', None), torch.int16) if d is not None) and tuple(a.shape) == shape
            if not ok or not a.is_cuda or not a.is_contiguous():
                raise ValueError('photometric: %s is a contiguous uint16 cuda tensor of shape %s, got %s %s' % (what, shape, a.dtype, tuple(a.shape)))
            return a
        a = np.asarray(a)
        if a.dtype != np.uint16 or tuple(a.shape) != shape:
            raise ValueError('photometric: %s is uint16 %s, got %s %s' % (what, shape, a.dtype, tuple(a.shape)))
        return torch.from_numpy(np.ascontiguousarray(a).view(np.int16)).to(_dev(device))
    r = None if response is None else table(response, 'response', (256,))
    g = None if gain is None else table(gain, 'gain', (h, w))
    oshape = tuple(t.shape)
    if out is None:
        out = torch.empty(oshape, dtype=torch.uint8, device=_dev(device))
    elif not (isinstance(out, torch.Tensor) and out.is_cuda and out.dtype == torch.uint8 and tuple(out.shape) == oshape):
        raise ValueError('photometric: out must be a uint8 cuda tensor of shape %s' % (oshape,))
    ob = out if batched else out.unsqueeze(0)
    if (n and not ob[0].is_contiguous()) or (n > 1 and ob.stride(0) < h * w):
        raise ValueError('photometric: every image of out must be contiguous')
    in_stride = tb.stride(0) if n > 1 else h * w
    out_stride = ob.stride(0) if n > 1 else h * w
    with torch.cuda.device(device):
        N.check(N.lib().av_photometric(N.dptr(tb), N.dptr(ob), n, w, h, in_stride, out_stride, None if r is None else N.dptr(r),
                                       None if g is None else N.dptr(g), N.current_stream()))
    return out


def to_gray8_range(img, scale='auto', window=None, clip=(100, 100), min_span=256, pool=1, index=None, out=None, work=None, device=0):
    mode, lo, hi, ppm_lo, ppm_hi, span = N.gray16_range_settings(scale, window, clip, min_span)
    if mode == N.AV_GRAY16_SHIFT:
        raise ValueError("to_gray8_range: scale is 'window' or 'auto' (ops.to_gray8 is the shift)")
    t = torch.as_tensor(img)
    if t.dtype not in (torch.uint16, torch.int16) or t.dim() not in (2, 3):
        raise ValueError('to_gray8_range: images are torch.uint16 / torch.int16 [n, h, w] or [h, w], got %s %s' % (t.dtype, tuple(t.shape)))
    t = t.to(_dev(device))
    batched = t.dim() == 3
    tb = t if batched else t.unsqueeze(0)
    n, h, w = tb.shape
    if pool not in (1, 2) or n % pool:
        raise ValueError('to_gray8_range: pool is 1 or 2 and divides the number of images (%d), got %r' % (n, pool))
    if (n and not tb[0].is_contiguous()) or (n > 1 and tb.stride(0) < h * w):
        tb = tb.contiguous()
    groups = n // pool
    oshape = tuple(t.shape)
    if out is None:
        if index is not None:
            raise ValueError('to_gray8_range: an index needs `out`')
        out = torch.empty(oshape, dtype=torch.uint8, device=_dev(device))
    elif not (isinstance(out, torch.Tensor) and out.is_cuda and out.dtype == torch.uint8 and (
            tuple(out.shape) == oshape if index is None else out.dim() == 3 and tuple(out.shape[1:]) == (h, w))):
        raise ValueError('to_gray8_range: out must be a uint8 cuda tensor of shape %s' % (oshape if index is None else ('m', h, w),))
    ob = out if out.dim() == 3 else out.unsqueeze(0)
    if (ob.shape[0] and not ob[0].is_contiguous()) or (ob.shape[0] > 1 and ob.stride(0) < h * w):
        raise ValueError('to_gray8_range: every image of out must be contiguous')
    first = None
    if index is not None:
        idx = [int(v) for v in index]
        if len(idx) != groups or any(e >= 0 and (e + 1) * pool > ob.shape[0] for e in idx):
            raise ValueError('to_gray8_range: index has one entry per group (%d), each negative or inside out (%d images)' % (groups, ob.shape[0]))
        last = {e: g for g, e in enumerate(idx)}
        first = torch.tensor([e if e >= 0 and last[e] == g else -1 for g, e in enumerate(idx)], dtype=torch.int32, device=_dev(device))
    if work is not None and not (isinstance(work, torch.Tensor) and work.is_cuda and work.dtype == torch.int32 and work.is_contiguous()
                                 and work.numel() >= groups * N.AV_GRAY16_WORK_WORDS):
        raise ValueError('to_gray8_range: work is a contiguous torch.int32 cuda tensor of at least %d elements' % (groups * N.AV_GRAY16_WORK_WORDS))
    ranges = torch.full((groups, 2), -1, dtype=torch.int32, device=_dev(device))
    in_stride = (tb.stride(0) if n > 1 else h * w) * tb.element_size()
    out_stride = ob.stride(0) if ob.shape[0] > 1 else h * w
    with torch.cuda.device(device):
        N.check(N.lib().av_to_gray8_range(N.dptr(tb), in_stride, n, w, h, mode, lo, hi, ppm_lo, ppm_hi, span, pool,
                                          None if first is None else N.dptr(first), N.dptr(ob), out_stride, N.dptr(ranges),
                                          None if work is None else N.dptr(work), N.current_stream()))
    return out, ranges
```

Baseline: 199,400.

## Slim pyramid kernels with magic-number division, packed u16 column filter, and restructured L2/L3

Replaces integer divisions in pyramid tile indexing with precomputed magic multipliers and simplifies the stereo-pair image mapping. The level-0 tile load now uses one thread per 16-byte chunk, with reflection only on edge tiles. Horizontal and vertical Gaussian passes use udot4 and packed 16-bit vector math. The fused L2/L3 kernel gets a new LDS layout with padded borders and a shared padded-store helper. It also adds an API to build levels without writing level 0, plus profiling scripts, at the cost of more complex edge-case handling.

```diff
diff --git a/include/airvision.h b/include/airvision.h
--- a/include/airvision.h
+++ b/include/airvision.h
@@ -35,6 +35,8 @@
 
 int av_pyramid_build(const uint8_t* img_dev, int64_t img_stride, int n_img, int w, int h, int levels,
                      uint8_t* pyr_dev, int64_t pyr_stride, void* stream);
+int av_pyramid_build_levels(const uint8_t* img_dev, int64_t img_stride, int n_img, int w, int h, int levels,
+                            uint8_t* pyr_dev, int64_t pyr_stride, void* stream);
 
 int av_lk_track(const uint8_t* pyrI_dev, const uint8_t* pyrJ_dev, int64_t pyr_stride, int n_set,
                 int w, int h, int levels,
diff --git a/profiles/pyramid_diet/census.py b/profiles/pyramid_diet/census.py
--- /dev/null
+++ b/profiles/pyramid_diet/census.py
@@ -0,0 +1,60 @@
+import re
+import sys
+
+
+def kind(op):
+    if op.startswith('v_'):
+        return 'valu'
+    if op.startswith('ds_'):
+        return 'lds'
+    if op.startswith(('global_', 'buffer_', 'flat_', 'scratch_')):
+        return 'vmem'
+    if op.startswith('s_'):
+        return 'salu'
+    return None
+
+
+def census(path, want=('pyr_l0l1_kernel', 'pyr_l2l3_kernel')):
+    lines = open(path).read().split('\n')
+    out = []
+    i = 0
+    while i < len(lines):
+        m = re.match(r'^(_Z\w+):', lines[i])
+        if not m or not any(w in m.group(1) for w in want):
+            i += 1
+            continue
+        name = m.group(1)
+        body = []
+        i += 1
+        while i < len(lines) and not lines[i].startswith('\t.end_amdhsa_kernel') and not re.match(r'^\s*s_endpgm', lines[i]):
+            body.append(lines[i])
+            i += 1
+        while i < len(lines) and not lines[i].startswith('\t.size') and not re.match(r'^\.Lfunc_end', lines[i]):
+            body.append(lines[i])
+            i += 1
+        tot = {'valu': 0, 'lds': 0, 'vmem': 0, 'salu': 0}
+        per, order, cur = {}, [], None
+        for l in body:
+            lm = re.match(r'^\.L(BB\w+):(.*)$', l)
+            if lm:
+                hm = re.search(r'Header=(BB\w+)', lm.group(2))
+                cur = lm.group(1) if 'Loop Header' in lm.group(2) else (hm.group(1) if hm else None)
+                if cur and cur not in per:
+                    per[cur] = {'valu': 0, 'lds': 0, 'vmem': 0, 'salu': 0}
+                    order.append(cur)
+                continue
+            t = l.strip().split()
+            if t and kind(t[0]):
+                tot[kind(t[0])] += 1
+                if cur:
+                    per[cur][kind(t[0])] += 1
+        loops = [(h, k, per[h]) for k, h in enumerate(order)]
+        out.append((name, tot, loops))
+    return out
+
+
+if __name__ == '__main__':
+    for name, tot, loops in census(sys.argv[1]):
+        print('%s: VALU %d  LDS %d  VMEM %d  SALU %d' % (name, tot['valu'], tot['lds'], tot['vmem'], tot['salu']))
+        for lab, at, c in sorted(loops, key=lambda x: x[1]):
+            print('    loop %-12s VALU %4d  LDS %3d  VMEM %3d' % (lab, c['valu'], c['lds'], c['vmem']))
diff --git a/profiles/pyramid_diet/copy_baseline.py b/profiles/pyramid_diet/copy_baseline.py
--- /dev/null
+++ b/profiles/pyramid_diet/copy_baseline.py
@@ -0,0 +1,33 @@
+import json
+import sys
+
+import torch
+
+sys.path.insert(0, __file__.rsplit('/profiles/', 1)[0])
+from uav_airvision_amd import ops
+
+w, h, streams = 752, 480, 2048
+lay = ops.pyramid_layout(w, h, 4)
+B = 16
+padded = [lay.pitch[l] * (lay.h[l] + 2 * B) for l in range(4)]
+read = w * h + padded[1]
+written = padded[1] + padded[2] + padded[3]
+total = (read + written) * 2 * streams
+n = total // 2
+src = torch.empty(n, dtype=torch.uint8, device='cuda')
+dst = torch.empty(n, dtype=torch.uint8, device='cuda')
+src.zero_()
+for _ in range(5):
+    dst.copy_(src)
+ms = []
+for _ in range(20):
+    e0, e1 = torch.cuda.Event(enable_timing=True), torch.cuda.Event(enable_timing=True)
+    e0.record()
+    dst.copy_(src)
+    e1.record()
+    e1.synchronize()
+    ms.append(e0.elapsed_time(e1))
+ms.sort()
+print(json.dumps({'read_per_image': read, 'written_per_image': written, 'bytes_moved_per_step': total, 'copy_bytes': n,
+                  'copy_ms_median': ms[len(ms) // 2], 'copy_ms_min': ms[0], 'copy_ms_max': ms[-1],
+                  'tb_per_s_median': total / (ms[len(ms) // 2] * 1e-3) / 1e12}))
diff --git a/uav_airvision_amd/_native.py b/uav_airvision_amd/_native.py
--- a/uav_airvision_amd/_native.py
+++ b/uav_airvision_amd/_native.py
@@ -178,6 +178,7 @@
     'av_device_count': (C.c_int, []),
     'av_pyramid_layout': (C.c_int, [C.c_int, C.c_int, C.c_int, C.POINTER(PyrLayout)]),
     'av_pyramid_build': (C.c_int, [_P, C.c_int64, C.c_int, C.c_int, C.c_int, C.c_int, _P, C.c_int64, _P]),
+    'av_pyramid_build_levels': (C.c_int, [_P, C.c_int64, C.c_int, C.c_int, C.c_int, C.c_int, _P, C.c_int64, _P]),
     'av_lk_track': (C.c_int, [_P, _P, C.c_int64, C.c_int, C.c_int, C.c_int, C.c_int, _P, _P, _P, _P, C.c_int,
                               C.c_int, C.c_int, C.c_double, C.c_double, _P]),
     'av_fast_detect': (C.c_int, [_P, C.c_int64, _P, C.c_int64, C.c_int, C.c_int, C.c_int, C.c_int, _P, _P, C.c_int, _P]),
diff --git a/uav_airvision_amd/csrc/pyramid.hip b/uav_airvision_amd/csrc/pyramid.hip
--- a/uav_airvision_amd/csrc/pyramid.hip
+++ b/uav_airvision_amd/csrc/pyramid.hip
@@ -15,13 +15,45 @@
     int slot0, slot1;
     PyrGeom g;
     int n_img, tiles_x, tiles_y;
+    uint32_t per_magic, tx_magic;
+    uint32_t m23[6];
     const int* index;
 };
 
+inline uint32_t pyr_magic(uint32_t d, uint64_t n_max) { return (d >= 2 && n_max * d < (1ull << 32)) ? 0xFFFFFFFFu / d + 1u : 0u; }
+__device__ __forceinline__ int pyr_div(int n, int d, uint32_t m) { return m ? (int)__umulhi((uint32_t)n, m) : n / d; }
+
 __device__ __forceinline__ void pyr_entry(const PyrArgs& a, int img, int& s, int& cam)
 {
-    s = img / a.imgs_per_stream; cam = img - s * a.imgs_per_stream;
+    const bool two = a.imgs_per_stream == 2;
+    s = two ? img >> 1 : img; cam = two ? img & 1 : 0;
     if (a.index) s = a.index[s];
+}
+
+typedef unsigned short pyr_u16x2 __attribute__((ext_vector_type(2)));
+typedef uint32_t pyr_u32x4 __attribute__((ext_vector_type(4)));
+typedef pyr_u32x4 pyr_u32x4_a4 __attribute__((aligned(4)));
+__device__ __forceinline__ void pyr_row4(uint32_t dx, uint32_t dy, uint32_t dz, uint32_t dw, uint32_t& p01, uint32_t& p23)
+{
+    const uint32_t W4 = 0x04060401u;
+    const uint32_t h0 = __builtin_amdgcn_udot4(__builtin_amdgcn_alignbyte(dy, dx, 2), W4, (dy >> 16) & 0xFF, false);
+    const uint32_t h1 = __builtin_amdgcn_udot4(dy, W4, dz & 0xFF, false);
+    const uint32_t h2 = __builtin_amdgcn_udot4(__builtin_amdgcn_alignbyte(dz, dy, 2), W4, (dz >> 16) & 0xFF, false);
+    const uint32_t h3 = __builtin_amdgcn_udot4(dz, W4, dw & 0xFF, false);
+    p01 = h0 | (h1 << 16); p23 = h2 | (h3 << 16);
+}
+__device__ __forceinline__ pyr_u16x2 pyr_col2(uint32_t r0, uint32_t r1, uint32_t r2, uint32_t r3, uint32_t r4)
+{
+    const pyr_u16x2 a0 = __builtin_bit_cast(pyr_u16x2, r0), a1 = __builtin_bit_cast(pyr_u16x2, r1), a2 = __builtin_bit_cast(pyr_u16x2, r2),
+                    a3 = __builtin_bit_cast(pyr_u16x2, r3), a4 = __builtin_bit_cast(pyr_u16x2, r4);
+    const pyr_u16x2 six = {6, 6}, half = {128, 128}, two = {2, 2}, eight = {8, 8};
+    return (a2 * six + half + ((a1 + a3) << two) + (a0 + a4)) >> eight;
+}
+__device__ __forceinline__ uint32_t pyr_col4(const uint32_t (&p01)[5], const uint32_t (&p23)[5])
+{
+    const uint32_t lo = __builtin_bit_cast(uint32_t, pyr_col2(p01[0], p01[1], p01[2], p01[3], p01[4]));
+    const uint32_t hi = __builtin_bit_cast(uint32_t, pyr_col2(p23[0], p23[1], p23[2], p23[3], p23[4]));
+    return __builtin_amdgcn_perm(hi, lo, 0x06040200u);
 }
 
 __device__ __forceinline__ uint8_t* pyr_of(const PyrArgs& a, int img)
@@ -76,10 +108,11 @@
     const int w1 = a.g.w[1], h1 = a.g.h[1], pitch1 = a.g.pitch[1];
     const int tid = threadIdx.x;
     const int L = blockIdx.x, wg = L >> 3, per = a.tiles_x * a.tiles_y;
-    const int img = (L & 7) + 8 * (wg / per);
+    const int grp = pyr_div(wg, per, a.per_magic);
+    const int img = (L & 7) + 8 * grp;
     if (img >= a.n_img) return;
-    const int tile = wg % per;
-    const int by = tile / a.tiles_x, bx = tile - by * a.tiles_x;
+    const int tile = wg - grp * per;
+    const int by = pyr_div(tile, a.tiles_x, a.tx_magic), bx = tile - by * a.tiles_x;
     const int x0 = bx * FT_W, y0 = by * FT_H;
     int s, cam;
     pyr_entry(a, img, s, cam);
@@ -88,70 +121,60 @@
     uint8_t* d0 = base + a.g.off[0];
     uint8_t* d1 = base + a.g.off[1];
     uint32_t* srcw = reinterpret_cast<uint32_t*>(src);
-
-    const bool al16 = ((a.img_stride & 15) == 0) && ((reinterpret_cast<uintptr_t>(in) & 15) == 0);
+    const bool top = y0 == 0, bot = y0 + FT_H >= h, left = x0 == 0, right = x0 + FT_W >= w;
+    const bool ragged = x0 + FT_W > w;
+
     {
-        constexpr int NIT = ((FT_H + 4) * 10 + 255) / 256;
-        uint4 q4[NIT]; uint32_t hv[NIT]; int kind[NIT], rr[NIT], jj[NIT];
+        constexpr int ROWS = FT_H + 4, NIT = (ROWS + 31) / 32;
+        static_assert(2 * ROWS <= 256, "one thread per halo dword");
+        const int j = tid & 7, r0 = tid >> 3;
+        const int gx = x0 + 16 * j;
+        const bool in_img = !ragged || gx < w;
+        uint32_t ro[NIT];
 #pragma unroll
         for (int u = 0; u < NIT; ++u) {
-            const int i = tid + 256 * u;
-            const bool valid = i < (FT_H + 4) * 10;
-            const int r = valid ? i / 10 : 0, j = valid ? i - r * 10 : 0;
-            rr[u] = r; jj[u] = j;
-            kind[u] = valid ? 3 : 0; hv[u] = 0; q4[u] = make_uint4(0, 0, 0, 0);
-        }
-        if (al16) {
-#pragma unroll
-            for (int u = 0; u < NIT; ++u) {
-                const int r = rr[u], j = jj[u];
-                const uint8_t* row = in + (size_t)av_reflect101(y0 - 2 + r, h) * w;
-                const int gx = x0 + 16 * j, gh = j == 8 ? x0 - 4 : x0 + FT_W;
-                const bool ok16 = kind[u] != 0 && j < 8 && gx + 16 <= w;
-                const bool okh = kind[u] != 0 && j >= 8 && gh >= 0 && gh + 4 <= w;
-                q4[u] = *reinterpret_cast<const uint4*>(ok16 ? row + gx : in);
-                hv[u] = *reinterpret_cast<const uint32_t*>(okh ? row + gh : in);
-                kind[u] = ok16 ? 1 : (okh ? 2 : kind[u]);
+            int y = y0 - 2 + r0 + 32 * u;
+            if (top || bot) y = av_reflect101(min(y, h + 1), h);
+            ro[u] = (uint32_t)(y * w);
+        }
+        const int hr = tid >> 1, gh = (tid & 1) ? x0 + FT_W : x0 - 4;
+        const bool hval = tid < 2 * ROWS, hin = gh >= 0 && gh + 4 <= w;
+        int hy = y0 - 2 + hr;
+        if (top || bot) hy = av_reflect101(min(hy, h + 1), h);
+        const uint8_t* hrow = in + (uint32_t)(hy * w);
+        uint32_t hv = 0;
+        pyr_u32x4 q4[NIT];
+        if (hval && hin) hv = *reinterpret_cast<const uint32_t*>(hrow + gh);
+        if (in_img) {
+#pragma unroll
+            for (int u = 0; u < NIT; ++u)
+                if (u < NIT - 1 || r0 + 32 * u < ROWS) q4[u] = *reinterpret_cast<const pyr_u32x4_a4*>(in + (ro[u] + (uint32_t)gx));
+        } else {
+#pragma unroll
+            for (int u = 0; u < NIT; ++u)
+                if (u < NIT - 1 || r0 + 32 * u < ROWS) {
+                    const uint8_t* row = in + ro[u];
+                    uint32_t v[4] = {0, 0, 0, 0};
+#pragma unroll
+                    for (int b = 0; b < 16; ++b) { int x = av_reflect101(gx + b, w); x = min(max(x, 0), w - 1); v[b >> 2] |= (uint32_t)row[x] << (8 * (b & 3)); }
+                    q4[u] = pyr_u32x4{v[0], v[1], v[2], v[3]};
+                }
+        }
+        if (hval && !hin) {
+#pragma unroll
+            for (int b = 0; b < 4; ++b) { int x = av_reflect101(gh + b, w); x = min(max(x, 0), w - 1); hv |= (uint32_t)hrow[x] << (8 * b); }
+        }
+        if (hval) srcw[hr * (FT_LP / 4) + ((tid & 1) ? FT_LP / 4 - 1 : 0)] = hv;
+#pragma unroll
+        for (int u = 0; u < NIT; ++u)
+            if (u < NIT - 1 || r0 + 32 * u < ROWS) {
+                uint32_t* dst = srcw + (r0 + 32 * u) * (FT_LP / 4) + 1 + 4 * j;
+                dst[0] = q4[u].x; dst[1] = q4[u].y; dst[2] = q4[u].z; dst[3] = q4[u].w;
             }
-        }
-#pragma unroll
-        for (int u = 0; u < NIT; ++u) {
-            const int r = rr[u], j = jj[u];
-            if (kind[u] == 1) {
-                uint32_t* dst = srcw + r * (FT_LP / 4) + 1 + 4 * j;
-                dst[0] = q4[u].x; dst[1] = q4[u].y; dst[2] = q4[u].z; dst[3] = q4[u].w;
-            } else if (kind[u] == 2) {
-                srcw[r * (FT_LP / 4) + (j == 8 ? 0 : FT_LP / 4 - 1)] = hv[u];
-            } else if (kind[u] == 3) {
-                const uint8_t* row = in + (size_t)av_reflect101(y0 - 2 + r, h) * w;
-                if (j < 8) {
-                    const int gx = x0 + 16 * j;
-                    uint32_t v[4];
-#pragma unroll
-                    for (int d = 0; d < 4; ++d) {
-                        if (gx + 4 * d + 4 <= w) v[d] = *reinterpret_cast<const uint32_t*>(row + gx + 4 * d);
-                        else {
-                            v[d] = 0;
-#pragma unroll
-                            for (int b = 0; b < 4; ++b) { int x = av_reflect101(gx + 4 * d + b, w); x = min(max(x, 0), w - 1); v[d] |= (uint32_t)row[x] << (8 * b); }
-                        }
-                    }
-                    uint32_t* dst = srcw + r * (FT_LP / 4) + 1 + 4 * j;
-                    dst[0] = v[0]; dst[1] = v[1]; dst[2] = v[2]; dst[3] = v[3];
-                } else {
-                    const int gx = j == 8 ? x0 - 4 : x0 + FT_W;
-                    uint32_t v = 0;
-#pragma unroll
-                    for (int b = 0; b < 4; ++b) { int x = av_reflect101(gx + b, w); x = min(max(x, 0), w - 1); v |= (uint32_t)row[x] << (8 * b); }
-                    srcw[r * (FT_LP / 4) + (j == 8 ? 0 : FT_LP / 4 - 1)] = v;
-                }
-            }
-        }
     }
     __syncthreads();
 
     if (WRITE_L0) {
-        const bool top = y0 == 0, bot = y0 + FT_H >= h, left = x0 == 0, right = x0 + FT_W >= w;
         const int tw = min(FT_W, w - x0);
         const int nrow = FT_H + (top ? AV_PYR_BORDER : 0) + (bot ? AV_PYR_BORDER : 0);
         const int nch_in = (tw + 15) >> 4;
@@ -189,43 +212,64 @@
         const int r = i / (FT_W / 8), xq = i - r * (FT_W / 8);
         const uint2 lo = *reinterpret_cast<const uint2*>(src + r * FT_LP + 8 * xq);
         const uint2 hi = *reinterpret_cast<const uint2*>(src + r * FT_LP + 8 * xq + 8);
-        const uint32_t dx_ = lo.x, dy_ = lo.y, dz_ = hi.x, dw_ = hi.y;
-        const uint32_t t0 = __builtin_amdgcn_alignbyte(dy_, dx_, 2), t1 = dy_, t2 = __builtin_amdgcn_alignbyte(dz_, dy_, 2), t3 = dz_;
-        const uint32_t W4 = 0x04060401u;
-        const uint32_t h0 = __builtin_amdgcn_udot4(t0, W4, (dy_ >> 16) & 0xFF, false);
-        const uint32_t h1_ = __builtin_amdgcn_udot4(t1, W4, dz_ & 0xFF, false);
-        const uint32_t h2 = __builtin_amdgcn_udot4(t2, W4, (dz_ >> 16) & 0xFF, false);
-        const uint32_t h3 = __builtin_amdgcn_udot4(t3, W4, dw_ & 0xFF, false);
-        *reinterpret_cast<uint2*>(hs + r * (FT_W / 2) + 4 * xq) = make_uint2(h0 | (h1_ << 16), h2 | (h3 << 16));
+        uint32_t p01, p23;
+        pyr_row4(lo.x, lo.y, hi.x, hi.y, p01, p23);
+        *reinterpret_cast<uint2*>(hs + r * (FT_W / 2) + 4 * xq) = make_uint2(p01, p23);
     }
     __syncthreads();
     for (int t_ = tid; t_ < (FT_H / 2) * (FT_W / 8); t_ += 256) {
         const int yo = t_ >> 4, xq = t_ & 15;
-        uint32_t out = 0;
         const uint16_t* c = hs + (2 * yo) * (FT_W / 2) + 4 * xq;
-#pragma unroll
-        for (int k = 0; k < 4; ++k) {
-            const int v = (int)c[k] + (int)c[4 * (FT_W / 2) + k] + 4 * ((int)c[(FT_W / 2) + k] + (int)c[3 * (FT_W / 2) + k]) + 6 * (int)c[2 * (FT_W / 2) + k];
-            out |= (uint32_t)((v + 128) >> 8) << (8 * k);
-        }
+        uint32_t p01[5], p23[5];
+#pragma unroll
+        for (int k = 0; k < 5; ++k) {
+            const uint2 v = *reinterpret_cast<const uint2*>(c + k * (FT_W / 2));
+            p01[k] = v.x; p23[k] = v.y;
+        }
+        const uint32_t out = pyr_col4(p01, p23);
         *reinterpret_cast<uint32_t*>(l1t + yo * (FT_W / 2) + 4 * xq) = out;
         const int x1 = x0 / 2 + 4 * xq, y1 = y0 / 2 + yo;
         if (x1 < w1 && y1 < h1) *reinterpret_cast<uint32_t*>(d1 + (size_t)(y1 + AV_PYR_BORDER) * pitch1 + (x1 + AV_PYR_BORDER)) = out;
     }
     const int X1 = x0 / 2, Y1 = y0 / 2;
-    const bool band = X1 <= AV_PYR_BORDER || X1 + FT_W / 2 >= w1 - AV_PYR_BORDER - 1 || Y1 <= AV_PYR_BORDER || Y1 + FT_H / 2 >= h1 - AV_PYR_BORDER - 1;
-    if (band) {
+    const int tx1 = min(X1 + FT_W / 2, w1), ty1 = min(Y1 + FT_H / 2, h1);
+    const bool hasL = X1 == 0, hasR = tx1 - 1 >= w1 - 1 - AV_PYR_BORDER;
+    const int rlo[3] = {Y1, max(Y1, 1), max(Y1, h1 - 1 - AV_PYR_BORDER)};
+    const int rhi[3] = {ty1 - 1, min(ty1 - 1, AV_PYR_BORDER), min(ty1 - 1, h1 - 2)};
+    if (hasL || hasR || rlo[1] <= rhi[1] || rlo[2] <= rhi[2]) {
         __syncthreads();
-        for (int i = tid; i < (FT_H / 2) * (FT_W / 2); i += 256) {
-            const int yo = i / (FT_W / 2), xo = i - yo * (FT_W / 2);
-            const int x1 = X1 + xo, y1 = Y1 + yo;
-            if (x1 >= w1 || y1 >= h1) continue;
-            const uint8_t v = l1t[i];
-            const int xm = (x1 >= 1 && x1 <= AV_PYR_BORDER) ? -x1 : ((x1 >= w1 - 1 - AV_PYR_BORDER && x1 <= w1 - 2) ? 2 * (w1 - 1) - x1 : INT_MIN);
-            const int ym = (y1 >= 1 && y1 <= AV_PYR_BORDER) ? -y1 : ((y1 >= h1 - 1 - AV_PYR_BORDER && y1 <= h1 - 2) ? 2 * (h1 - 1) - y1 : INT_MIN);
-            if (xm != INT_MIN) d1[(size_t)(y1 + AV_PYR_BORDER) * pitch1 + (xm + AV_PYR_BORDER)] = v;
-            if (ym != INT_MIN) d1[(size_t)(ym + AV_PYR_BORDER) * pitch1 + (x1 + AV_PYR_BORDER)] = v;
-            if (xm != INT_MIN && ym != INT_MIN) d1[(size_t)(ym + AV_PYR_BORDER) * pitch1 + (xm + AV_PYR_BORDER)] = v;
+        const uint32_t* l1w = reinterpret_cast<const uint32_t*>(l1t);
+#pragma unroll
+        for (int rk = 0; rk < 3; ++rk) {
+            const int ya = rlo[rk], nr = rhi[rk] - ya + 1;
+            if (nr <= 0) continue;
+            if (rk != 0) {
+                for (int i = tid; i < nr * (FT_W / 8); i += 256) {
+                    const int yy = ya + (i >> 4), q = i & 15;
+                    const int yd = rk == 1 ? -yy : 2 * (h1 - 1) - yy;
+                    if (X1 + 4 * q < tx1)
+                        *reinterpret_cast<uint32_t*>(d1 + (size_t)(yd + AV_PYR_BORDER) * pitch1 + (X1 + 4 * q + AV_PYR_BORDER)) = l1w[(yy - Y1) * (FT_W / 8) + q];
+                }
+            }
+#pragma unroll
+            for (int ck = 1; ck < 3; ++ck) {
+                if (!(ck == 1 ? hasL : hasR)) continue;
+                for (int i = tid; i < nr * 4; i += 256) {
+                    const int yy = ya + (i >> 2), k = i & 3;
+                    const int yd = rk == 0 ? yy : (rk == 1 ? -yy : 2 * (h1 - 1) - yy);
+                    const int xd = ck == 1 ? 4 * k - AV_PYR_BORDER : w1 + 4 * k;
+                    const int xs = ck == 1 ? -xd : 2 * (w1 - 1) - xd;
+                    const uint8_t* sp = l1t + (yy - Y1) * (FT_W / 2) + (xs - X1);
+                    uint8_t* dp = d1 + (size_t)(yd + AV_PYR_BORDER) * pitch1 + (xd + AV_PYR_BORDER);
+                    if (xs < tx1 && xs - 3 >= X1) {
+                        *reinterpret_cast<uint32_t*>(dp) = (uint32_t)sp[0] | (uint32_t)sp[-1] << 8 | (uint32_t)sp[-2] << 16 | (uint32_t)sp[-3] << 24;
+                    } else {
+#pragma unroll
+                        for (int c = 0; c < 4; ++c)
+                            if (xs - c < tx1 && xs - c >= X1) dp[c] = sp[-c];
+                    }
+                }
+            }
         }
     }
 }
@@ -283,95 +327,92 @@
     *reinterpret_cast<uint32_t*>(dst + (size_t)yp * pitch + xq * 4) = out;
 }
 
+enum { L23_Q2 = 0, L23_Q3, L23_IN2, L23_FR2, L23_IN3, L23_FR3 };
+struct L23Layout { int q2, q3, lp2, lp3, l3_off, bytes; };
+__host__ __device__ inline L23Layout pyr_l23_layout(const PyrGeom& g)
+{
+    L23Layout l;
+    l.q2 = (g.w[2] + 3) >> 2; l.q3 = (g.w[3] + 3) >> 2;
+    l.lp2 = 8 * l.q3 + 8;
+    l.lp3 = 4 * l.q3;
+    l.l3_off = ((g.h[2] + 4) * l.lp2 + 15) & ~15;
+    l.bytes = l.l3_off + g.h[3] * l.lp3;
+    return l;
+}
+
+template <int T>
+__device__ __forceinline__ void pyr_store_padded(const uint8_t* l, int lp, int w, int h, uint8_t* d, int pitch, uint32_t m_in, uint32_t m_fr, int tid)
+{
+    const int ph = h + 2 * AV_PYR_BORDER, nin = w >> 2, nfr = (pitch >> 2) - nin;
+    for (int i = tid; i < nin * ph; i += T) {
+        const int yp = pyr_div(i, nin, m_in), q = i - yp * nin;
+        const int y = av_reflect101(yp - AV_PYR_BORDER, h);
+        *reinterpret_cast<uint32_t*>(d + yp * pitch + (AV_PYR_BORDER + 4 * q)) = *reinterpret_cast<const uint32_t*>(l + y * lp + 4 * q);
+    }
+    for (int i = tid; i < nfr * ph; i += T) {
+        const int yp = pyr_div(i, nfr, m_fr), q = i - yp * nfr;
+        const int y = av_reflect101(yp - AV_PYR_BORDER, h);
+        const int xs = q < 4 ? 4 * q - AV_PYR_BORDER : 4 * (nin + q - 4);
+        uint32_t out = 0;
+#pragma unroll
+        for (int c = 0; c < 4; ++c) { int x = av_reflect101(xs + c, w); x = min(max(x, 0), w - 1); out |= (uint32_t)l[y * lp + x] << (8 * c); }
+        *reinterpret_cast<uint32_t*>(d + yp * pitch + (xs + AV_PYR_BORDER)) = out;
+    }
+}
+
 template <int L23_T>
 __global__ __launch_bounds__(L23_T) void pyr_l2l3_kernel(PyrArgs a)
 {
-    extern __shared__ uint8_t lds23[];
-    const int w1 = a.g.w[1], p1 = a.g.pitch[1];
+    extern __shared__ __attribute__((aligned(16))) uint8_t lds23[];
+    const int p1 = a.g.pitch[1];
     const int w2 = a.g.w[2], h2 = a.g.h[2], p2 = a.g.pitch[2];
     const int w3 = a.g.w[3], h3 = a.g.h[3], p3 = a.g.pitch[3];
-    const int lp2 = (w2 + 3) & ~3, lp3 = (w3 + 3) & ~3;
-    uint8_t* l2 = lds23;
-    uint8_t* l3 = lds23 + (((size_t)h2 * lp2 + 15) & ~(size_t)15);
+    const L23Layout lay = pyr_l23_layout(a.g);
+    const int q2 = lay.q2, q3 = lay.q3, lp2 = lay.lp2, lp3 = lay.lp3;
+    uint8_t* l2 = lds23 + 2 * lp2 + 4;
+    uint8_t* l3 = lds23 + lay.l3_off;
     const int tid = threadIdx.x;
     uint8_t* base = pyr_of(a, blockIdx.x);
-    const uint8_t* s1 = base + a.g.off[1] + (size_t)AV_PYR_BORDER * p1 + AV_PYR_BORDER;
-    uint8_t* d2 = base + a.g.off[2];
-    uint8_t* d3 = base + a.g.off[3];
-    (void)w1;
-    const int q2 = lp2 >> 2;
+    const uint8_t* s1 = base + a.g.off[1] + (AV_PYR_BORDER - 2) * p1 + (AV_PYR_BORDER - 4);
     for (int i = tid; i < q2 * h2; i += L23_T) {
-        const int y = i / q2, x0 = (i - y * q2) * 4;
-        const uint8_t* r0 = s1 + (ptrdiff_t)(2 * y - 2) * p1;
-        int hs[4][5];
+        const int y = pyr_div(i, q2, a.m23[L23_Q2]), q = i - y * q2;
+        const uint8_t* r0 = s1 + (uint32_t)(2 * y * p1 + 8 * q);
+        uint32_t p01[5], p23[5];
 #pragma unroll
         for (int k = 0; k < 5; ++k) {
-            const uint4 d = *reinterpret_cast<const uint4*>(r0 + (size_t)k * p1 + 2 * x0 - 4);
-            const uint32_t t0 = __builtin_amdgcn_alignbyte(d.y, d.x, 2), t1 = d.y, t2 = __builtin_amdgcn_alignbyte(d.z, d.y, 2), t3 = d.z;
-            const uint32_t W4 = 0x04060401u;
-            hs[0][k] = (int)__builtin_amdgcn_udot4(t0, W4, (d.y >> 16) & 0xFF, false);
-            hs[1][k] = (int)__builtin_amdgcn_udot4(t1, W4, d.z & 0xFF, false);
-            hs[2][k] = (int)__builtin_amdgcn_udot4(t2, W4, (d.z >> 16) & 0xFF, false);
-            hs[3][k] = (int)__builtin_amdgcn_udot4(t3, W4, d.w & 0xFF, false);
-        }
-        uint32_t out = 0;
-#pragma unroll
-        for (int c = 0; c < 4; ++c) {
-            const int v = hs[c][0] + hs[c][4] + 4 * (hs[c][1] + hs[c][3]) + 6 * hs[c][2];
-            out |= (uint32_t)((v + 128) >> 8) << (8 * c);
-        }
-        *reinterpret_cast<uint32_t*>(l2 + y * lp2 + x0) = out;
+            const uint4 d = *reinterpret_cast<const uint4*>(r0 + k * p1);
+            pyr_row4(d.x, d.y, d.z, d.w, p01[k], p23[k]);
+        }
+        *reinterpret_cast<uint32_t*>(l2 + y * lp2 + 4 * q) = pyr_col4(p01, p23);
     }
     __syncthreads();
-    const int ph2 = h2 + 2 * AV_PYR_BORDER, pq2 = p2 >> 2;
-    for (int i = tid; i < pq2 * ph2; i += L23_T) {
-        const int yp = i / pq2, xq = i - yp * pq2;
-        const int y = av_reflect101(yp - AV_PYR_BORDER, h2);
-        uint32_t out = 0;
-        const int xs = xq * 4 - AV_PYR_BORDER;
-        if (xs >= 0 && xs + 4 <= w2) out = *reinterpret_cast<const uint32_t*>(l2 + y * lp2 + xs);
-        else {
-#pragma unroll
-            for (int c = 0; c < 4; ++c) { int x = av_reflect101(xs + c, w2); x = min(max(x, 0), w2 - 1); out |= (uint32_t)l2[y * lp2 + x] << (8 * c); }
-        }
-        *reinterpret_cast<uint32_t*>(d2 + (size_t)yp * p2 + xq * 4) = out;
-    }
-    const int q3 = lp3 >> 2;
-    for (int i = tid; i < q3 * h3; i += L23_T) {
-        const int y = i / q3, x0 = (i - y * q3) * 4;
-        uint32_t out = 0;
-#pragma unroll
-        for (int c = 0; c < 4; ++c) {
-            const int x = x0 + c;
-            int v = 0;
-            if (x < w3) {
-                int hsum[5];
-#pragma unroll
-                for (int k = 0; k < 5; ++k) {
-                    const uint8_t* r = l2 + av_reflect101(2 * y - 2 + k, h2) * lp2;
-                    const int xm2 = av_reflect101(2 * x - 2, w2), xm1 = av_reflect101(2 * x - 1, w2), xp1 = av_reflect101(2 * x + 1, w2), xp2 = av_reflect101(2 * x + 2, w2);
-                    hsum[k] = (int)r[xm2] + (int)r[xp2] + 4 * ((int)r[xm1] + (int)r[xp1]) + 6 * (int)r[2 * x];
-                }
-                v = (hsum[0] + hsum[4] + 4 * (hsum[1] + hsum[3]) + 6 * hsum[2] + 128) >> 8;
-            }
-            out |= (uint32_t)v << (8 * c);
-        }
-        *reinterpret_cast<uint32_t*>(l3 + y * lp3 + x0) = out;
+    for (int i = tid; i < 4 * h2; i += L23_T) {
+        const int y = i >> 2, c = i & 3;
+        const int xd = c < 2 ? c - 2 : w2 + c - 2;
+        l2[y * lp2 + xd] = l2[y * lp2 + av_reflect101(xd, w2)];
     }
     __syncthreads();
-    const int ph3 = h3 + 2 * AV_PYR_BORDER, pq3 = p3 >> 2;
-    for (int i = tid; i < pq3 * ph3; i += L23_T) {
-        const int yp = i / pq3, xq = i - yp * pq3;
-        const int y = av_reflect101(yp - AV_PYR_BORDER, h3);
-        uint32_t out = 0;
-        const int xs = xq * 4 - AV_PYR_BORDER;
-        if (xs >= 0 && xs + 4 <= w3) out = *reinterpret_cast<const uint32_t*>(l3 + y * lp3 + xs);
-        else {
-#pragma unroll
-            for (int c = 0; c < 4; ++c) { int x = av_reflect101(xs + c, w3); x = min(max(x, 0), w3 - 1); out |= (uint32_t)l3[y * lp3 + x] << (8 * c); }
-        }
-        *reinterpret_cast<uint32_t*>(d3 + (size_t)yp * p3 + xq * 4) = out;
-    }
+    for (int i = tid; i < (lp2 >> 2); i += L23_T) {
+        uint32_t* col = reinterpret_cast<uint32_t*>(lds23) + i;
+        const int dw = lp2 >> 2;
+        col[0] = col[4 * dw]; col[dw] = col[3 * dw];
+        col[(h2 + 2) * dw] = col[h2 * dw]; col[(h2 + 3) * dw] = col[(h2 - 1) * dw];
+    }
+    __syncthreads();
+    pyr_store_padded<L23_T>(l2, lp2, w2, h2, base + a.g.off[2], p2, a.m23[L23_IN2], a.m23[L23_FR2], tid);
+    for (int i = L23_T - 1 - tid; i < q3 * h3; i += L23_T) {
+        const int y = pyr_div(i, q3, a.m23[L23_Q3]), q = i - y * q3;
+        const uint8_t* r0 = lds23 + 2 * y * lp2 + 8 * q;
+        uint32_t p01[5], p23[5];
+#pragma unroll
+        for (int k = 0; k < 5; ++k) {
+            const uint2 lo = *reinterpret_cast<const uint2*>(r0 + k * lp2), hi = *reinterpret_cast<const uint2*>(r0 + k * lp2 + 8);
+            pyr_row4(lo.x, lo.y, hi.x, hi.y, p01[k], p23[k]);
+        }
+        *reinterpret_cast<uint32_t*>(l3 + y * lp3 + 4 * q) = pyr_col4(p01, p23);
+    }
+    __syncthreads();
+    pyr_store_padded<L23_T>(l3, lp3, w3, h3, base + a.g.off[3], p3, a.m23[L23_IN3], a.m23[L23_FR3], tid);
 }
 
 }
@@ -397,7 +438,8 @@
     a.img0 = img.base[0]; a.img1 = img.base[1]; a.img_stride = img.stride; a.imgs_per_stream = img.base[1] ? 2 : 1;
     a.pyr_base = pyr_base; a.stream_stride = stream_stride; a.slot_stride = slot_stride;
     a.slot0 = slot0; a.slot1 = slot1; a.g = g;
-    a.n_img = 0; a.tiles_x = 0; a.tiles_y = 0; a.index = img.map;
+    a.n_img = 0; a.tiles_x = 0; a.tiles_y = 0; a.per_magic = 0; a.tx_magic = 0; a.index = img.map;
+    memset(a.m23, 0, sizeof(a.m23));
     const int n_img = n_groups * a.imgs_per_stream;
     const int w = g.w[0], h = g.h[0];
     const int FT_H = ((h % FT_H_TALL) == 0 && h >= 2 * FT_H_TALL) ? FT_H_TALL : FT_H_BASE;
@@ -407,6 +449,7 @@
         const int tx = (w + FT_W - 1) / FT_W, ty = h / FT_H;
         a.n_img = n_img; a.tiles_x = tx; a.tiles_y = ty;
         dim3 grid((unsigned)(tx * ty) * 8u * (unsigned)((n_img + 7) / 8));
+        a.per_magic = pyr_magic((uint32_t)(tx * ty), grid.x >> 3); a.tx_magic = pyr_magic((uint32_t)tx, (uint64_t)(tx * ty));
         if (FT_H == FT_H_TALL) {
             if (write_level0) hipLaunchKernelGGL((pyr_l0l1_kernel<true, FT_H_TALL>), grid, dim3(256), 0, st, a);
             else { hipLaunchKernelGGL((pyr_l0l1_kernel<false, FT_H_TALL>), grid, dim3(256), 0, st, a); if (wrote_level0) *wrote_level0 = false; }
@@ -422,7 +465,8 @@
         AV_LAUNCH_CHECK();
     }
     const size_t lds23 = g.levels == 4 ? ((((size_t)g.h[2] * ((g.w[2] + 3) & ~3) + 15) & ~(size_t)15) + (size_t)g.h[3] * ((g.w[3] + 3) & ~3) + 16) : 0;
-    const bool fused23 = g.levels == 4 && lds23 <= 60 * 1024 && (g.pitch[1] & 3) == 0;
+    const L23Layout l23 = pyr_l23_layout(g);
+    const bool fused23 = g.levels == 4 && lds23 <= 60 * 1024 && (g.pitch[1] & 3) == 0 && l23.bytes <= 64 * 1024;
     int lbeg = fused ? 2 : 1;
     if (fused23) {
         if (!fused) {
@@ -431,7 +475,14 @@
             hipLaunchKernelGGL(pyr_down_kernel, grid, dim3(256), 0, st, a, 1);
             AV_LAUNCH_CHECK();
         }
-        hipLaunchKernelGGL(pyr_l2l3_kernel<1024>, dim3(n_img), dim3(1024), lds23, st, a);
+        for (int l = 2; l <= 3; ++l) {
+            const uint32_t ph = (uint32_t)(g.h[l] + 2 * AV_PYR_BORDER), nin = (uint32_t)(g.w[l] >> 2), nfr = (uint32_t)(g.pitch[l] >> 2) - nin;
+            const uint32_t q = (uint32_t)(l == 2 ? l23.q2 : l23.q3);
+            a.m23[l == 2 ? L23_Q2 : L23_Q3] = pyr_magic(q, (uint64_t)q * g.h[l]);
+            a.m23[l == 2 ? L23_IN2 : L23_IN3] = pyr_magic(nin, (uint64_t)nin * ph);
+            a.m23[l == 2 ? L23_FR2 : L23_FR3] = pyr_magic(nfr, (uint64_t)nfr * ph);
+        }
+        hipLaunchKernelGGL(pyr_l2l3_kernel<1024>, dim3(n_img), dim3(1024), (size_t)l23.bytes, st, a);
         AV_LAUNCH_CHECK();
         lbeg = g.levels;
     }
@@ -470,15 +521,27 @@
     return AV_OK;
 }
 
-AV_EXPORT int av_pyramid_build(const uint8_t* img_dev, int64_t img_stride, int n_img, int w, int h, int levels,
-                               uint8_t* pyr_dev, int64_t pyr_stride, void* stream)
+static int pyramid_build(const char* who, const uint8_t* img_dev, int64_t img_stride, int n_img, int w, int h, int levels,
+                         uint8_t* pyr_dev, int64_t pyr_stride, void* stream, bool write_level0)
 {
     av_pyr_layout lay;
     int rc = av_pyramid_layout(w, h, levels, &lay);
     if (rc) return rc;
     if (!img_dev || !pyr_dev || n_img < 0 || pyr_stride < lay.bytes || img_stride < (int64_t)w * h) {
-        av_set_error("av_pyramid_build: bad arguments");
+        av_set_error("%s: bad arguments", who);
         return AV_E_INVALID;
     }
-    return av_launch_pyramid(av_frames(img_dev, nullptr, img_stride), n_img, av_make_geom(lay), pyr_dev, pyr_stride, 0, 0, 0, (hipStream_t)stream);
-}
+    return av_launch_pyramid(av_frames(img_dev, nullptr, img_stride), n_img, av_make_geom(lay), pyr_dev, pyr_stride, 0, 0, 0, (hipStream_t)stream, write_level0);
+}
+
+AV_EXPORT int av_pyramid_build(const uint8_t* img_dev, int64_t img_stride, int n_img, int w, int h, int levels,
+                               uint8_t* pyr_dev, int64_t pyr_stride, void* stream)
+{
+    return pyramid_build("av_pyramid_build", img_dev, img_stride, n_img, w, h, levels, pyr_dev, pyr_stride, stream, true);
+}
+
+AV_EXPORT int av_pyramid_build_levels(const uint8_t* img_dev, int64_t img_stride, int n_img, int w, int h, int levels,
+                                      uint8_t* pyr_dev, int64_t pyr_stride, void* stream)
+{
+    return pyramid_build("av_pyramid_build_levels", img_dev, img_stride, n_img, w, h, levels, pyr_dev, pyr_stride, stream, false);
+}
diff --git a/uav_airvision_amd/ops.py b/uav_airvision_amd/ops.py
--- a/uav_airvision_amd/ops.py
+++ b/uav_airvision_amd/ops.py
@@ -16,17 +16,21 @@
     return lay
 
 
-def build_pyramids(images, levels, device=0):
+def build_pyramids(images, levels, device=0, write_level0=True, out=None):
     t = torch.as_tensor(images)
     if t.dim() == 2:
         t = t[None]
     t = t.to(_dev(device), dtype=torch.uint8).contiguous()
     n, h, w = t.shape
     lay = pyramid_layout(w, h, levels)
-    pyr = torch.empty((n, lay.bytes), dtype=torch.uint8, device=_dev(device))
-    with torch.cuda.device(device):
-        N.check(N.lib().av_pyramid_build(N.dptr(t), w * h, n, w, h, levels, N.dptr(pyr), lay.bytes, N.current_stream()))
-    return pyr, lay
+    if out is None:
+        out = torch.empty((n, lay.bytes), dtype=torch.uint8, device=_dev(device))
+    if out.dtype != torch.uint8 or tuple(out.shape) != (n, lay.bytes) or not out.is_contiguous() or out.device != t.device:
+        raise ValueError('out must be a contiguous uint8 tensor [%d, %d] on %s' % (n, lay.bytes, t.device))
+    build = N.lib().av_pyramid_build if write_level0 else N.lib().av_pyramid_build_levels
+    with torch.cuda.device(device):
+        N.check(build(N.dptr(t), w * h, n, w, h, levels, N.dptr(out), lay.bytes, N.current_stream()))
+    return out, lay
 
 
 def pyramid_level(pyr_row, lay, level, with_border=False):
```

New measurement: 203,600, median of 6. +2.1%, better.
